# mitake/k8s

Measured on AMD Instinct MI355X. Metric: images/sec ResNet-50 TfJob (train, synthetic ImageNet), higher is better.
Workload: dtype bf16; 1 GPU; model=resnet50-v1.5, global_batch=3072, per_gpu_batch=3072, image_size=224, parallelism=dp1, optimizer=fused SGD momentum 0.9 (HIP)

## Files before the change

k8s_amd/csrc/binding/batchnorm.cpp:

```cpp
#include "binding/common.h"

namespace k8s_amd::binding {
namespace {

int bn_channels(const Tensor& x, const char* name, bool mult8) {
  check_bf16_dense(x, -1, name);
  TORCH_CHECK(x.dim() >= 1 && x.size(-1) > 0, name, ": channels last");
  const int C = (int)x.size(-1);
  TORCH_CHECK(!mult8 || C % 8 == 0, "channels must be a multiple of 8");
  return C;
}
void check_affine(const Tensor& gamma, const Tensor& beta, const Tensor& run_mean, const Tensor& run_var, long C) {
  check_channel_f32(gamma, C, "gamma"); check_channel_f32(beta, C, "beta");
  check_channel_f32(run_mean, C, "run_mean"); check_channel_f32(run_var, C, "run_var");
}
void check_bwd_vectors(const Tensor& mean, const Tensor& invstd, const Tensor& gamma, const Tensor& beta,
                       const Tensor& dgamma, const Tensor& dbeta, long C) {
  check_channel_f32(mean, C, "mean"); check_channel_f32(invstd, C, "invstd");
  check_channel_f32(gamma, C, "gamma"); check_channel_f32(beta, C, "beta");
  check_channel_f32(dgamma, C, "dgamma"); check_channel_f32(dbeta, C, "dbeta");
}
void check_same_shape(const Tensor& t, const Tensor& x, const char* name) {
  check_bf16_dense(t, -1, name);
  TORCH_CHECK(t.sizes() == x.sizes(), name, " must have the shape of x");
}

Tensor relu_mask_for(const Tensor& x, bool want_mask) {
  return want_mask ? torch::empty({x.numel() / 8}, x.options().dtype(at::kByte)) : Tensor();
}

std::vector<Tensor> bn_fwd_impl(const Tensor& x, const OptTensor& res, const Tensor& gamma, const Tensor& beta,
                                const Tensor* sums, const Tensor& run_mean, const Tensor& run_var, bool training,
                                double momentum, double eps, bool relu, bool want_mask, bool want_sub2) {
  const int C = bn_channels(x, "x", true);
  const long M = x.numel() / C;
  check_affine(gamma, beta, run_mean, run_var, C);
  const int nrep = sums ? check_stat_sums(*sums, C, "sums", false) : 0;
  if (res) check_same_shape(*res, x, "res");
  TORCH_CHECK(!want_sub2 || x.dim() == 4, "want_sub2: contiguous NHWC x");
  auto y = torch::empty_like(x);
  auto mean = torch::empty({C}, gamma.options()), invstd = torch::empty({C}, gamma.options());
  auto params = torch::empty({2 * C}, gamma.options());
  Tensor mask = relu_mask_for(x, want_mask);
  uint8_t* mk = want_mask ? mask.data_ptr<uint8_t>() : nullptr;
  std::vector<Tensor> out = {y, mean, invstd};
  if (want_mask) out.push_back(mask);
  if (!sums) {
    Tensor work = training ? torch::empty({k8s_amd::bn_workspace_floats(M, C)}, gamma.options()) : mean;
    launch_bn_fwd(cbf(x), res ? cbf(*res) : nullptr, f32(gamma), f32(beta), bf(y), f32(mean), f32(invstd),
                  f32(run_mean), f32(run_var), f32(work), f32(params), M, C, (float)eps, (float)momentum, training,
                  relu, cur_stream(), mk);
    return out;
  }
  const int H = want_sub2 ? (int)x.size(1) : 1, W = want_sub2 ? (int)x.size(2) : 1;
  Tensor ysub = want_sub2 ? torch::empty({x.size(0), (H + 1) / 2, (W + 1) / 2, C}, x.options()) : Tensor();
  launch_bn_fwd_from_sums(cbf(x), res ? cbf(*res) : nullptr, f32(gamma), f32(beta), bf(y), f32(*sums), nrep, f32(mean),
                          f32(invstd), f32(run_mean), f32(run_var), f32(params), M, C, (float)eps, (float)momentum,
                          relu, cur_stream(), mk, want_sub2 ? bf(ysub) : nullptr, H, W);
  if (want_sub2) out.push_back(ysub);
  return out;
}
std::vector<Tensor> bn_fwd(Tensor x, OptTensor res, Tensor gamma, Tensor beta, Tensor run_mean, Tensor run_var,
                           bool training, double momentum, double eps, bool relu, bool want_mask) {
  return bn_fwd_impl(x, res, gamma, beta, nullptr, run_mean, run_var, training, momentum, eps, relu, want_mask, false);
}
std::vector<Tensor> bn_fwd_from_sums(Tensor x, OptTensor res, Tensor gamma, Tensor beta, Tensor sums, Tensor run_mean,
                                     Tensor run_var, double momentum, double eps, bool relu, bool want_mask,
                                     bool want_sub2) {
  return bn_fwd_impl(x, res, gamma, beta, &sums, run_mean, run_var, true, momentum, eps, relu, want_mask, want_sub2);
}

std::vector<Tensor> bn_fwd_from_sums_dual(Tensor x, Tensor sums, Tensor gamma, Tensor beta, Tensor run_mean,
                                          Tensor run_var, Tensor xr, Tensor sums_r, Tensor gamma_r, Tensor beta_r,
                                          Tensor run_mean_r, Tensor run_var_r, double momentum, double eps) {
  const int C = bn_channels(x, "x", true);
  const long M = x.numel() / C;
  check_same_shape(xr, x, "xr");
  check_affine(gamma, beta, run_mean, run_var, C);
  check_affine(gamma_r, beta_r, run_mean_r, run_var_r, C);
  const int nrep = check_stat_sums(sums, C, "sums", false), nrep_r = check_stat_sums(sums_r, C, "sums_r", false);
  auto y = torch::empty_like(x);
  auto mean = torch::empty({C}, gamma.options()), invstd = torch::empty({C}, gamma.options());
  auto mean_r = torch::empty({C}, gamma.options()), invstd_r = torch::empty({C}, gamma.options());
  auto params = torch::empty({2 * C}, gamma.options()), params_r = torch::empty({2 * C}, gamma.options());
  Tensor mask = relu_mask_for(x, true);
  launch_bn_fwd_from_sums_dual(cbf(x), f32(gamma), f32(beta), f32(sums), nrep, f32(mean), f32(invstd), f32(run_mean),
                               f32(run_var), f32(params), cbf(xr), f32(gamma_r), f32(beta_r), f32(sums_r), nrep_r,
                               f32(mean_r), f32(invstd_r), f32(run_mean_r), f32(run_var_r), f32(params_r), bf(y),
                               mask.data_ptr<uint8_t>(), M, C, (float)eps, (float)momentum, cur_stream());
  return {y, mean, invstd, mask, mean_r, invstd_r};
}

std::vector<Tensor> bn_finalize(Tensor sums, Tensor gamma, Tensor beta, Tensor run_mean, Tensor run_var,
                                int64_t count, double momentum, double eps) {
  const int C = (int)gamma.numel();
  check_affine(gamma, beta, run_mean, run_var, C);
  const int nrep = check_stat_sums(sums, C, "sums", false);
  auto mean = torch::empty({C}, gamma.options()), invstd = torch::empty({C}, gamma.options());
  auto params = torch::empty({2 * C}, gamma.options());
  launch_bn_finalize_sums(f32(gamma), f32(beta), f32(sums), nrep, f32(mean), f32(invstd), f32(run_mean), f32(run_var),
                          f32(params), (long)count, C, (float)eps, (float)momentum, cur_stream());
  return {mean, invstd, params};
}

std::vector<Tensor> bn_relu_maxpool(Tensor x, Tensor sums, Tensor gamma, Tensor beta, Tensor run_mean, Tensor run_var,
                                    double momentum, double eps, bool want_link) {
  check_bf16_dense(x, 4, "x");
  const int N = x.size(0), H = x.size(1), W = x.size(2), C = x.size(3);
  TORCH_CHECK(C > 0 && C % 8 == 0 && 256 % (C / 8) == 0, "C / 8 must divide 256");
  check_affine(gamma, beta, run_mean, run_var, C);
  const int nrep = check_stat_sums(sums, C, "sums", false);
  const int Ho = (H + 1) / 2, Wo = (W + 1) / 2;
  auto y = torch::empty({N, Ho, Wo, C}, x.options());
  auto idx = torch::empty({N, Ho, Wo, C}, x.options().dtype(at::kByte));
  auto mean = torch::empty({C}, gamma.options()), invstd = torch::empty({C}, gamma.options());
  auto params = torch::empty({2 * C}, gamma.options());
  Tensor xarg, ybits;
  if (want_link) {
    xarg = torch::empty({N, Ho, Wo, C}, x.options());
    ybits = torch::empty({(long)N * Ho * Wo * C / 8}, x.options().dtype(at::kByte));
  }
  launch_bn_relu_maxpool_fwd(cbf(x), f32(gamma), f32(beta), f32(sums), nrep, f32(mean), f32(invstd), f32(run_mean),
                             f32(run_var), f32(params), bf(y), idx.data_ptr<uint8_t>(), N, H, W, C, (float)eps,
                             (float)momentum, cur_stream(), want_link ? bf(xarg) : nullptr,
                             want_link ? ybits.data_ptr<uint8_t>() : nullptr);
  if (want_link) return {y, idx, mean, invstd, xarg, ybits};
  return {y, idx, mean, invstd};
}

Tensor pool_bn_bwd_impl(const Tensor& dpool, const Tensor& idx, const Tensor& x, const Tensor& mean,
                        const Tensor& invstd, const Tensor& gamma, const Tensor& beta, const Tensor& dgamma,
                        const Tensor& dbeta, const Tensor* sums) {
  check_bf16_dense(x, 4, "x");
  check_bf16_dense(dpool, 4, "dpool");
  check_cuda(idx, "idx"); check_dtype(idx, at::kByte, "idx");
  const int N = x.size(0), H = x.size(1), W = x.size(2), C = x.size(3);
  TORCH_CHECK(dpool.sizes() == idx.sizes() && dpool.size(0) == N && dpool.size(1) == (H + 1) / 2 &&
                  dpool.size(2) == (W + 1) / 2 && dpool.size(3) == C, "dpool / idx shape mismatch");
  check_bwd_vectors(mean, invstd, gamma, beta, dgamma, dbeta, C);
  const int nrep = sums ? check_stat_sums(*sums, C, "sums", true) : 0;
  auto dx = torch::empty_like(x);
  auto params = torch::empty({4 * C}, gamma.options());
  if (sums) {
    launch_pool_bn_bwd_from_sums(cbf(dpool), idx.data_ptr<uint8_t>(), cbf(x), f32(mean), f32(invstd), f32(gamma),
                                 f32(beta), bf(dx), f32(dgamma), f32(dbeta), f32(*sums), nrep, f32(params), N, H, W, C,
                                 cur_stream());
    return dx;
  }
  auto work = torch::empty({k8s_amd::pool_bn_workspace_floats(C)}, gamma.options());
  launch_pool_bn_bwd(cbf(dpool), idx.data_ptr<uint8_t>(), cbf(x), f32(mean), f32(invstd), f32(gamma), f32(beta), bf(dx),
                     f32(dgamma), f32(dbeta), f32(work), f32(params), N, H, W, C, cur_stream());
  return dx;
}
Tensor pool_bn_bwd_from_sums(Tensor dpool, Tensor idx, Tensor x, Tensor mean, Tensor invstd, Tensor gamma,
                             Tensor beta, Tensor dgamma, Tensor dbeta, Tensor sums) {
  return pool_bn_bwd_impl(dpool, idx, x, mean, invstd, gamma, beta, dgamma, dbeta, &sums);
}
Tensor pool_bn_bwd(Tensor dpool, Tensor idx, Tensor x, Tensor mean, Tensor invstd, Tensor gamma, Tensor beta,
                   Tensor dgamma, Tensor dbeta) {
  return pool_bn_bwd_impl(dpool, idx, x, mean, invstd, gamma, beta, dgamma, dbeta, nullptr);
}

std::vector<Tensor> bn_bwd_impl(const Tensor& dy, const Tensor& x, const OptTensor& y, const Tensor& mean,
                                const Tensor& invstd, const Tensor& gamma, const Tensor& beta, bool relu_x,
                                const Tensor& dgamma, const Tensor& dbeta, bool want_dres, const OptTensor& mask,
                                const Tensor* sums) {
  const int C = bn_channels(x, "x", false);
  const long M = x.numel() / C;
  check_same_shape(dy, x, "dy");
  check_bwd_vectors(mean, invstd, gamma, beta, dgamma, dbeta, C);
  const bool has_mask = mask && mask->defined();
  TORCH_CHECK(!(relu_x && (y || has_mask)) && !(y && has_mask), "relu_x, y and the packed mask are exclusive");
  const uint8_t* mk = has_mask ? check_bit_mask(*mask, x.numel(), "mask") : nullptr;
  const int nrep = sums ? check_stat_sums(*sums, C, "sums", false) : 0;
  Tensor ymask;
  if (y) {
    check_same_shape(*y, x, "y");
    TORCH_CHECK(x.numel() % 8 == 0, "y: a multiple of 8 elements to pack");
    ymask = relu_mask_for(x, true);
    launch_relu_mask(cbf(*y), ymask.data_ptr<uint8_t>(), x.numel() / 8, cur_stream());
    mk = ymask.data_ptr<uint8_t>();
  }
  auto dx = torch::empty_like(x);
  Tensor dres = want_dres ? torch::empty_like(x) : Tensor();
  uint16_t* dr = want_dres ? bf(dres) : nullptr;
  auto params = torch::empty({4 * C}, gamma.options());
  if (sums && mk) {
    launch_bn_bwd_from_sums(cbf(dy), cbf(x), mk, f32(*sums), nrep, f32(mean), f32(invstd), f32(gamma), f32(beta),
                            bf(dx), dr, f32(dgamma), f32(dbeta), f32(params), M, C, cur_stream());
  } else if (sums) {
    launch_bn_bwd_relu_from_sums(cbf(dy), cbf(x), f32(*sums), nrep, f32(mean), f32(invstd), f32(gamma), f32(beta),
                                 bf(dx), f32(dgamma), f32(dbeta), f32(params), M, C, cur_stream());
  } else {
    auto work = torch::empty({k8s_amd::bn_workspace_floats(M, C)}, gamma.options());
    launch_bn_bwd(cbf(dy), cbf(x), f32(mean), f32(invstd), f32(gamma), f32(beta), relu_x, bf(dx), dr, f32(dgamma),
                  f32(dbeta), f32(work), f32(params), M, C, cur_stream(), mk);
  }
  return {dx, dres};
}
std::vector<Tensor> bn_bwd(Tensor dy, Tensor x, OptTensor y, Tensor mean, Tensor invstd, Tensor gamma, Tensor beta,
                           bool relu_x, Tensor dgamma, Tensor dbeta, bool want_dres, OptTensor mask) {
  return bn_bwd_impl(dy, x, y, mean, invstd, gamma, beta, relu_x, dgamma, dbeta, want_dres, mask, nullptr);
}
std::vector<Tensor> bn_bwd_relu_from_sums(Tensor dy, Tensor x, Tensor sums, Tensor mean, Tensor invstd, Tensor gamma,
                                          Tensor beta, Tensor dgamma, Tensor dbeta) {
  return {bn_bwd_impl(dy, x, {}, mean, invstd, gamma, beta, true, dgamma, dbeta, false, {}, &sums)[0]};
}
std::vector<Tensor> bn_bwd_from_sums(Tensor dy, Tensor x, Tensor mask, Tensor sums, Tensor mean, Tensor invstd,
                                     Tensor gamma, Tensor beta, Tensor dgamma, Tensor dbeta, bool want_dres) {
  return bn_bwd_impl(dy, x, {}, mean, invstd, gamma, beta, false, dgamma, dbeta, want_dres, mask, &sums);
}

std::vector<Tensor> bn_bwd_dual_impl(const Tensor& dy, const Tensor& mask, const Tensor& x, const Tensor& mean,
                                     const Tensor& invstd, const Tensor& gamma, const Tensor& beta,
                                     const Tensor& dgamma, const Tensor& dbeta, const Tensor* sums, const Tensor& x2,
                                     const Tensor& mean2, const Tensor& invstd2, const Tensor& gamma2,
                                     const Tensor& beta2, const Tensor& dgamma2, const Tensor& dbeta2,
                                     const Tensor* sums2) {
  const int C = bn_channels(x, "x", !sums);
  const long M = x.numel() / C;
  check_same_shape(dy, x, "dy");
  check_same_shape(x2, x, "x2");
  check_bwd_vectors(mean, invstd, gamma, beta, dgamma, dbeta, C);
  check_bwd_vectors(mean2, invstd2, gamma2, beta2, dgamma2, dbeta2, C);
  const uint8_t* mk = check_bit_mask(mask, x.numel(), "mask");
  const int nrep = sums ? check_stat_sums(*sums, C, "sums", false) : 0;
  TORCH_CHECK(!sums || check_stat_sums(*sums2, C, "sums2", false) == nrep, "sums / sums2: the same replica count");
  auto dx = torch::empty_like(x), dx2 = torch::empty_like(x);
  auto params = torch::empty({4 * C}, gamma.options()), params2 = torch::empty({4 * C}, gamma.options());
  if (sums) {
    launch_bn_bwd_dual_from_sums(cbf(dy), mk, cbf(x), f32(*sums), nrep, f32(mean), f32(invstd), f32(gamma), f32(beta),
                                 bf(dx), f32(dgamma), f32(dbeta), f32(params), cbf(x2), f32(*sums2), f32(mean2),
                                 f32(invstd2), f32(gamma2), f32(beta2), bf(dx2), f32(dgamma2), f32(dbeta2),
                                 f32(params2), M, C, cur_stream());
    return {dx, dx2};
  }
  auto work = torch::empty({k8s_amd::bn_workspace_floats(M, C)}, gamma.options());
  auto work2 = torch::empty({k8s_amd::bn_workspace_floats(M, C)}, gamma.options());
  launch_bn_bwd_dual(cbf(dy), mk, cbf(x), f32(mean), f32(invstd), f32(gamma), f32(beta), bf(dx), f32(dgamma),
                     f32(dbeta), f32(work), f32(params), cbf(x2), f32(mean2), f32(invstd2), f32(gamma2), f32(beta2),
                     bf(dx2), f32(dgamma2), f32(dbeta2), f32(work2), f32(params2), M, C, cur_stream());
  return {dx, dx2};
}
std::vector<Tensor> bn_bwd_dual(Tensor dy, Tensor mask, Tensor x, Tensor mean, Tensor invstd, Tensor gamma,
                                Tensor beta, Tensor dgamma, Tensor dbeta, Tensor x2, Tensor mean2, Tensor invstd2,
                                Tensor gamma2, Tensor beta2, Tensor dgamma2, Tensor dbeta2) {
  return bn_bwd_dual_impl(dy, mask, x, mean, invstd, gamma, beta, dgamma, dbeta, nullptr, x2, mean2, invstd2, gamma2,
                          beta2, dgamma2, dbeta2, nullptr);
}
std::vector<Tensor> bn_bwd_dual_from_sums(Tensor dy, Tensor mask, Tensor x, Tensor mean, Tensor invstd, Tensor gamma,
                                          Tensor beta, Tensor dgamma, Tensor dbeta, Tensor sums, Tensor x2,
                                          Tensor mean2, Tensor invstd2, Tensor gamma2, Tensor beta2, Tensor dgamma2,
                                          Tensor dbeta2, Tensor sums2) {
  return bn_bwd_dual_impl(dy, mask, x, mean, invstd, gamma, beta, dgamma, dbeta, &sums, x2, mean2, invstd2, gamma2,
                          beta2, dgamma2, dbeta2, &sums2);
}

}

void bind_batchnorm(pybind11::module_& m) {
  m.def("bn_fwd", &bn_fwd, "x"_a, "res"_a, "gamma"_a, "beta"_a, "run_mean"_a, "run_var"_a, "training"_a, "momentum"_a,
        "eps"_a, "relu"_a, "want_mask"_a = false);
  m.def("bn_bwd", &bn_bwd, "dy"_a, "x"_a, "y"_a, "mean"_a, "invstd"_a, "gamma"_a, "beta"_a, "relu_x"_a, "dgamma"_a,
        "dbeta"_a, "want_dres"_a, "mask"_a = py::none());
  m.def("bn_fwd_from_sums", &bn_fwd_from_sums, "x"_a, "res"_a, "gamma"_a, "beta"_a, "sums"_a, "run_mean"_a, "run_var"_a,
        "momentum"_a, "eps"_a, "relu"_a, "want_mask"_a = false, "want_sub2"_a = false);
  m.def("bn_bwd_dual", &bn_bwd_dual, "both BatchNorm backwards of bn_fwd_from_sums_dual from one masked dy");
  m.def("bn_fwd_from_sums_dual", &bn_fwd_from_sums_dual, "relu(BN(x) + BN_r(xr)), statistics from conv sums");
  m.def("bn_finalize", &bn_finalize, "sums"_a, "gamma"_a, "beta"_a, "run_mean"_a, "run_var"_a, "count"_a, "momentum"_a,
        "eps"_a);
  m.def("bn_bwd_relu_from_sums", &bn_bwd_relu_from_sums, "relu_x BatchNorm backward from a producer's sums");
  m.def("bn_bwd_from_sums", &bn_bwd_from_sums, "BatchNorm backward from a producer's reduction sums (final + apply)");
  m.def("bn_bwd_dual_from_sums", &bn_bwd_dual_from_sums, "bn_bwd_dual from a producer's reduction sums");
  m.def("bn_relu_maxpool", &bn_relu_maxpool, "x"_a, "sums"_a, "gamma"_a, "beta"_a, "run_mean"_a, "run_var"_a,
        "momentum"_a, "eps"_a, "want_link"_a = false);
  m.def("pool_bn_bwd_from_sums", &pool_bn_bwd_from_sums);
  m.def("pool_bn_bwd", &pool_bn_bwd, "dpool"_a, "idx"_a, "x"_a, "mean"_a, "invstd"_a, "gamma"_a, "beta"_a, "dgamma"_a,
        "dbeta"_a);
}

}
```

k8s_amd/csrc/binding/conv.cpp:

```cpp
#include "binding/common.h"

namespace k8s_amd::binding {
namespace {

int conv_out(int in, int k, int st, int pad, int dil) { return (in + 2 * pad - dil * (k - 1) - 1) / st + 1; }

struct ConvGeom {
  int N, H, W, C, K, R, S;
};
ConvGeom conv_geom(const Tensor& x, const Tensor& w) {
  TORCH_CHECK(x.dim() == 4 && w.dim() == 4, "x [N,H,W,C], w [K,R,S,C]");
  ConvGeom g{(int)x.size(0), (int)x.size(1), (int)x.size(2), (int)x.size(3),
             (int)w.size(0), (int)w.size(1), (int)w.size(2)};
  TORCH_CHECK(w.size(3) == g.C, "channel mismatch");
  TORCH_CHECK(g.C % 8 == 0 && g.K % 8 == 0, "implicit-GEMM conv needs C % 8 == 0 and K % 8 == 0");
  return g;
}
Tensor conv_fwd(Tensor x, Tensor w, int64_t stride, int64_t pad, int64_t dil, bool out_f32, OptTensor bias, int64_t act,
                OptTensor stats, OptTensor xform) {
  check_bf16(x, "x"); check_bf16(w, "w");
  const auto [N, H, W, C, K, R, S] = conv_geom(x, w);
  TORCH_CHECK(stride >= 1 && dil >= 1, "conv_fwd: stride >= 1, dilation >= 1");
  const int Ho = conv_out(H, R, stride, pad, dil), Wo = conv_out(W, S, stride, pad, dil);
  if (bias) check_channel_f32(*bias, K, "bias");
  if (stats) check_stat_sums(*stats, K, "stats", true);
  const float* xf = xform_ptr(xform, C);
  if (xf) TORCH_CHECK(C % 64 == 0 && !out_f32 && !bias && act == 0,
                      "normalize-on-load convolution: C % 64 == 0, bf16 output, no bias / activation");
  auto y = torch::empty({N, Ho, Wo, K}, x.options().dtype(out_f32 ? at::kFloat : at::kBFloat16));
  launch_conv_fwd(cbf(x), cbf(w), y.data_ptr(), out_f32, N, H, W, C, K, R, S, (int)stride, (int)pad, (int)dil, Ho, Wo,
                  optf(bias), (int)act, 0, stats ? f32(*stats) : nullptr, cur_stream(), nullptr, xf);
  return y;
}

Tensor conv_infer(Tensor x, Tensor w, int64_t stride, int64_t pad, Tensor scale, Tensor shift, OptTensor res,
                  bool relu, OptTensor out) {
  check_bf16_dense(x, 4, "x"); check_bf16_dense(w, 4, "w");
  const auto [N, H, W, C, K, R, S] = conv_geom(x, w);
  TORCH_CHECK(stride >= 1 && pad >= 0, "conv_infer: stride >= 1, pad >= 0");
  check_channel_f32(scale, K, "scale"); check_channel_f32(shift, K, "shift");
  TORCH_CHECK(H + 2 * pad >= R && W + 2 * pad >= S, "conv_infer: the filter does not fit the padded image");
  const int Ho = conv_out(H, R, stride, pad, 1), Wo = conv_out(W, S, stride, pad, 1);
  TORCH_CHECK((long)N * Ho * Wo < (1L << 31), "conv_infer: fewer than 2^31 output pixels");
  const std::vector<int64_t> oshape{N, Ho, Wo, K};
  if (out) {
    check_bf16_dense(*out, 4, "out");
    TORCH_CHECK(out->sizes().vec() == oshape, "out must be [N, Ho, Wo, K]");
  }
  if (res) {
    check_bf16_dense(*res, 4, "res");
    TORCH_CHECK(res->sizes().vec() == oshape, "res must have the output's shape [N, Ho, Wo, K]");
  }
  Tensor y = out ? *out : torch::empty(oshape, x.options());
  launch_conv_infer(cbf(x), cbf(w), bf(y), N, H, W, C, K, R, S, (int)stride, (int)pad, Ho, Wo, f32(scale), f32(shift),
                    res ? cbf(*res) : nullptr, relu, cur_stream());
  return y;
}

void conv_fwd_subgrid(Tensor x, Tensor w, int64_t pad, int64_t Hs, int64_t Ws, Tensor out, int64_t stride, int64_t a,
                      int64_t b, bool accumulate, OptTensor bn_x, OptTensor bn_mask, OptTensor bn_mean,
                      OptTensor bn_sums, OptTensor bn_gamma, OptTensor bn_beta, OptTensor bn_invstd) {
  check_bf16(x, "x"); check_bf16(w, "w"); check_bf16(out, "out");
  const auto [N, H, W, C, K, R, S] = conv_geom(x, w);
  TORCH_CHECK(out.dim() == 4 && out.size(0) == N && out.size(3) == K, "out shape");
  const int OH = out.size(1), OW = out.size(2);
  TORCH_CHECK(stride >= 1 && a >= 0 && a < stride && b >= 0 && b < stride, "parity out of range");
  TORCH_CHECK(Hs >= 1 && Ws >= 1 && (Hs - 1) * stride + a < OH && (Ws - 1) * stride + b < OW,
              "sub-grid exceeds the output image");
  k8s_amd::SubGrid sg{OH, OW, (int)stride, (int)a, (int)b};
  k8s_amd::BnBwdSums bb;
  if (bn_sums) {
    TORCH_CHECK(bn_x && bn_mean, "bn sums: bn_x and bn_mean");
    TORCH_CHECK(bn_mask ? accumulate : !accumulate,
                "bn sums: bn_mask + accumulate (a correction) or bn_gamma / bn_beta / bn_invstd + a plain store");
    TORCH_CHECK(bn_x->sizes() == out.sizes(), "bn_x: the shape of out");
    bb = bn_bwd_sums(*bn_x, *bn_mean, *bn_sums, bn_mask, bn_gamma, bn_beta, bn_invstd, {}, {}, {});
  }
  launch_conv_fwd(cbf(x), cbf(w), out.data_ptr(), false, N, H, W, C, K, R, S, 1, (int)pad, 1, (int)Hs, (int)Ws, nullptr,
                  0, accumulate ? 1 : 0, nullptr, cur_stream(), &sg, nullptr, bn_sums ? &bb : nullptr);
}

Tensor conv3x3_dgrad_bnstats(Tensor gy, Tensor wt, Tensor x, Tensor gamma, Tensor beta, Tensor mean, Tensor invstd,
                             Tensor sums) {
  check_bf16_dense(gy, 4, "gy"); check_bf16_dense(wt, 4, "wt"); check_bf16_dense(x, 4, "x");
  const int N = (int)gy.size(0), H = (int)gy.size(1), W = (int)gy.size(2), Kc = (int)gy.size(3);
  const int C = (int)wt.size(0);
  TORCH_CHECK(wt.size(1) == 3 && wt.size(2) == 3 && wt.size(3) == Kc, "wt: [C, 3, 3, K]");
  TORCH_CHECK(x.size(0) == N && x.size(1) == H && x.size(2) == W && x.size(3) == C, "x: the shape of dx");
  TORCH_CHECK(k8s_amd::conv3x3_eligible(H, W, Kc, C, 3, 3, 1, 1, 1), "conv3x3_dgrad_bnstats: outside the kernel");
  const k8s_amd::BnBwdSums bb = bn_bwd_sums(x, mean, sums, {}, gamma, beta, invstd, {}, {}, {});
  Tensor dx = torch::empty({N, H, W, C}, gy.options());
  launch_conv3x3(cbf(gy), cbf(wt), bf(dx), nullptr, nullptr, N, H, W, Kc, C, cur_stream(), &bb);
  return dx;
}

Tensor bwd1x1_fused(Tensor gy, Tensor x, Tensor w, Tensor xform, Tensor gamma, Tensor beta, Tensor mean, Tensor invstd,
                    Tensor dw, Tensor sums, bool accumulate) {
  check_bf16_dense(gy, 2, "gy"); check_bf16_dense(x, 2, "x"); check_bf16_dense(w, 2, "w");
  const long M = gy.size(0), K = gy.size(1), C = x.size(1);
  TORCH_CHECK(x.size(0) == M && w.size(0) == K && w.size(1) == C, "shapes: gy [M, K], x [M, C], w [K, C]");
  TORCH_CHECK(k8s_amd::bwd1x1_fused_ok(M, (int)C, (int)K),
              "bwd1x1_fused: (C, K) = (64, 256) or (128, 512), 1 <= M < 2^31");
  check_cuda(dw, "dw"); check_dtype(dw, at::kFloat, "dw"); check_aligned(dw, "dw");
  TORCH_CHECK(dw.numel() == K * C, "dw must have K * C fp32 elements");
  check_channel_f32(xform, 2 * C, "xform (BatchNorm scale | shift)");
  const k8s_amd::BnBwdSums bb = bn_bwd_sums(x, mean, sums, {}, gamma, beta, invstd, {}, {}, {});
  Tensor dz = torch::empty({M, C}, gy.options());
  launch_bwd1x1_fused(cbf(gy), cbf(x), cbf(w), f32(xform), bb.gamma, bb.beta, bb.mean, bb.invstd, bf(dz), f32(dw),
                      bb.sums, M, (int)C, (int)K, accumulate, cur_stream());
  return dz;
}

void conv_wgrad(Tensor x, Tensor dy, Tensor dw, int64_t stride, int64_t pad, int64_t dil, int64_t splits,
                bool accumulate, OptTensor xform) {
  check_bf16(x, "x"); check_bf16(dy, "dy");
  check_cuda(dw, "dw"); check_dtype(dw, at::kFloat, "dw");
  const auto [N, H, W, C, K, R, S] = conv_geom(x, dw);
  TORCH_CHECK(stride >= 1 && dil >= 1, "conv_wgrad: stride >= 1, dilation >= 1");
  const int Ho = conv_out(H, R, stride, pad, dil), Wo = conv_out(W, S, stride, pad, dil);
  TORCH_CHECK(dy.dim() == 4 && dy.size(0) == N && dy.size(1) == Ho && dy.size(2) == Wo && dy.size(3) == K,
              "dy shape mismatch");
  const float* xf = xform_ptr(xform, C);
  if (dil == 1 && Ho == H && Wo == W && H == W && k8s_amd::wgrad3x3_tiled_ok(C, K, R, S, (int)stride, (int)pad, W)) {
    auto wsp = torch::empty({k8s_amd::wgrad3x3_tiled_workspace(N, H, W, C)}, dw.options());
    launch_wgrad3x3_tiled(cbf(x), cbf(dy), f32(wsp), f32(dw), N, H, W, C, accumulate, cur_stream(), xf);
    return;
  }
  if (!xf && dil == 1 && k8s_amd::wgrad_stream_eligible(N, Ho, Wo, C, K, R, S)) {
    launch_wgrad_stream(cbf(x), cbf(dy), f32(dw), N, H, W, C, K, R, S, (int)stride, (int)pad, Ho, Wo, accumulate,
                        cur_stream());
    return;
  }
  if (xf) TORCH_CHECK(C % 64 == 0, "normalize-on-load weight gradient needs C % 64 == 0");
  int sp = splits <= 0 ? k8s_amd::gemm_choose_splits(K, R * S * C, N * Ho * Wo) : (int)splits;
  Tensor ws;
  if (sp > 1) ws = torch::empty({k8s_amd::gemm_splitk_workspace(K, R * S * C, sp)}, dw.options());
  launch_conv_wgrad(cbf(x), cbf(dy), f32(dw), N, H, W, C, K, R, S, (int)stride, (int)pad, (int)dil, Ho, Wo, sp,
                    accumulate, sp > 1 ? f32(ws) : nullptr, cur_stream(), xf);
}

std::vector<Tensor> conv_dgrad_wsub(Tensor w, std::vector<std::vector<int64_t>> taps) {
  check_bf16(w, "w");
  TORCH_CHECK(w.dim() == 4, "w [K,R,S,C]");
  const int K = w.size(0), R = w.size(1), S = w.size(2), C = w.size(3);
  TORCH_CHECK(!taps.empty() && taps.size() <= 16, "1-16 parities");
  k8s_amd::DgradTaps t{};
  long off = 0;
  std::vector<int64_t> offs;
  for (size_t p = 0; p < taps.size(); ++p) {
    TORCH_CHECK(!taps[p].empty() && taps[p].size() <= 16, "1-16 taps per parity");
    t.n[p] = (int)taps[p].size();
    t.off[p] = off;
    offs.push_back(off);
    for (size_t i = 0; i < taps[p].size(); ++i) {
      TORCH_CHECK(taps[p][i] >= 0 && taps[p][i] < R * S, "tap index out of range");
      t.rs[p][i] = (int)taps[p][i];
    }
    off += (long)C * t.n[p] * K;
    off = (off + 7) / 8 * 8;
  }
  auto out = torch::empty({off}, w.options());
  launch_conv_dgrad_wsub(cbf(w), bf(out), K, R * S, C, t, (int)taps.size(), cur_stream());
  return {out, torch::tensor(offs)};
}
Tensor conv_dgrad_wtrans(Tensor w) {
  check_bf16(w, "w");
  TORCH_CHECK(w.dim() == 4, "w [K,R,S,C]");
  const int K = w.size(0), R = w.size(1), S = w.size(2), C = w.size(3);
  auto w2 = torch::empty({C, R, S, K}, w.options());
  launch_conv_dgrad_wtrans(cbf(w), bf(w2), K, R, S, C, cur_stream());
  return w2;
}

}

void bind_conv(pybind11::module_& m) {
  m.def("conv_fwd", &conv_fwd, "x"_a, "w"_a, "stride"_a, "pad"_a, "dil"_a, "out_f32"_a, "bias"_a, "act"_a, "stats"_a,
        "xform"_a = py::none());
  m.def("conv_infer", &conv_infer, "x"_a, "w"_a, "stride"_a, "pad"_a, "scale"_a, "shift"_a, "res"_a = py::none(),
        "relu"_a = true, "out"_a = py::none());
  m.def("conv3x3_staged_ok", [](int H, int W, int C, int K, int R, int S, int stride, int pad) {
    return k8s_amd::conv3x3_eligible(H, W, C, K, R, S, stride, pad, 1) &&
           k8s_amd::conv3x3_eligible(H, W, K, C, R, S, stride, pad, 1) &&
           k8s_amd::wgrad3x3_tiled_ok(C, K, R, S, stride, pad, W);
  });
  m.def("conv3x3_dgrad_bnstats", &conv3x3_dgrad_bnstats,
        "3x3 stride-1 data gradient with the BatchNorm-backward sums of a relu(BN(x)) input (conv3x3.hip)");
  m.def("conv_fwd_subgrid", &conv_fwd_subgrid, "x"_a, "w"_a, "pad"_a, "Hs"_a, "Ws"_a, "out"_a, "stride"_a, "a"_a, "b"_a,
        "accumulate"_a = false, "bn_x"_a = py::none(), "bn_mask"_a = py::none(), "bn_mean"_a = py::none(),
        "bn_sums"_a = py::none(), "bn_gamma"_a = py::none(), "bn_beta"_a = py::none(), "bn_invstd"_a = py::none());
  m.def("conv_wgrad", &conv_wgrad, "x"_a, "dy"_a, "dw"_a, "stride"_a, "pad"_a, "dil"_a, "splits"_a, "accumulate"_a,
        "xform"_a = py::none());
  m.def("bwd1x1_fused", &bwd1x1_fused, "gy"_a, "x"_a, "w"_a, "xform"_a, "gamma"_a, "beta"_a, "mean"_a, "invstd"_a,
        "dw"_a, "sums"_a, "accumulate"_a,
        "1x1 data gradient, normalize-on-load weight gradient and BatchNorm-backward sums in one pass (bwd1x1_fused.hip)");
  m.def("bwd1x1_fused_ok", [](int64_t M, int64_t C, int64_t K) {
    return C <= 1024 && K <= 4096 && k8s_amd::bwd1x1_fused_ok(M, (int)C, (int)K);
  }, "M"_a, "C"_a, "K"_a, "whether bwd1x1_fused takes this shape");
  m.def("wgrad_stream_eligible",&k8s_amd::wgrad_stream_eligible, "tall-K weight-gradient kernel takes this shape");
  m.def("conv_dgrad_wtrans", &conv_dgrad_wtrans);
  m.def("conv_dgrad_wsub", &conv_dgrad_wsub);
}

}
```

k8s_amd/csrc/kernels/batchnorm.hip:

```cpp
#include <cstdlib>
#include <stdexcept>

#include "common.h"
#include "launchers.h"

namespace k8s_amd {


constexpr int BN_THREADS = 256;

struct BnGeom {
  int cgroups;
  int tpr;
  int rows_per_iter;
  int grid_y;
};

static inline BnGeom bn_geom(int C, long M) {
  BnGeom g;
  g.cgroups = C / 8;
  g.tpr = g.cgroups < BN_THREADS ? g.cgroups : BN_THREADS;
  const long cus = planner_cus();
  long nbx = M / 64;
  nbx = nbx < 1 ? 1 : (nbx > 4 * cus ? 4 * cus : nbx);
// ... 508 lines not shown


__global__ void __launch_bounds__(BN_THREADS) bn_relu_maxpool_fwd_kernel(
    const uint16_t* __restrict__ x, const float* __restrict__ params, uint16_t* __restrict__ y,
    uint8_t* __restrict__ idx, int H, int W, int C, int Ho, int Wo, int total, FastDiv fcv, FastDiv fWo, FastDiv fHo,
    uint16_t* __restrict__ xarg, uint8_t* __restrict__ ybits) {
  const int e = blockIdx.x * BN_THREADS + threadIdx.x;
  if (e >= total) return;
  const int cv = C >> 3;
  const int t = fcv.div(e);
  const int c = (e - t * cv) * 8;
  const int t2 = fWo.div(t);
  const int wo = t - t2 * Wo;
  const int n = fHo.div(t2);
  const int ho = t2 - n * Ho;
  const int h0 = 2 * ho - 1, w0 = 2 * wo - 1;
  float sc[8], sh[8];
  load_f8(params + c, sc);
  load_f8(params + C + c, sh);
  bf16x8_t v[9];
#pragma unroll
  for (int dh = 0; dh < 3; ++dh)
#pragma unroll
    for (int dw = 0; dw < 3; ++dw) {
      const int h = min(max(h0 + dh, 0), H - 1), w = min(max(w0 + dw, 0), W - 1);
      v[dh * 3 + dw] = *reinterpret_cast<const bf16x8_t*>(x + (((long)n * H + h) * W + w) * C + c);
    }
  float best[8];
  uint32_t arg[8];
  bf16x8_t bx = bf16x8_t{0, 0, 0, 0, 0, 0, 0, 0};
#pragma unroll
  for (int j = 0; j < 8; ++j) {
    best[j] = -INFINITY;
    arg[j] = 255;
  }
#pragma unroll
  for (int dh = 0; dh < 3; ++dh)
#pragma unroll
    for (int dw = 0; dw < 3; ++dw) {
      if ((unsigned)(h0 + dh) >= (unsigned)H || (unsigned)(w0 + dw) >= (unsigned)W) continue;
#pragma unroll
      for (int j = 0; j < 8; ++j) {
        const float z = bf2f(f2bf(fmaxf(__builtin_fmaf(bf2f((uint16_t)v[dh * 3 + dw][j]), sc[j], sh[j]), 0.f)));
        if (z > best[j] || (z != z && best[j] == best[j])) {
          best[j] = z;
          arg[j] = (uint32_t)(dh * 3 + dw);
          bx[j] = v[dh * 3 + dw][j];
        }
      }
    }
  store8(y + (long)e * 8, best);
  uint64_t packed = 0;
#pragma unroll
  for (int j = 0; j < 8; ++j) packed |= (uint64_t)arg[j] << (8 * j);
  *reinterpret_cast<uint64_t*>(idx + (long)e * 8) = packed;
  if (xarg) {
    *reinterpret_cast<bf16x8_t*>(xarg + (long)e * 8) = bx;
    uint32_t bits = 0;
#pragma unroll
    for (int j = 0; j < 8; ++j) bits |= (best[j] > 0.f ? 1u : 0u) << j;
    ybits[e] = (uint8_t)bits;
  }
}

struct PoolCell {
  float dz[2][2][8];
};
__device__ __forceinline__ void pool_cell_grad(const uint16_t* __restrict__ dpool, const uint8_t* __restrict__ idx,
                                               int n, int kc, int jc, int c, int C, int Ho, int Wo, PoolCell& pc) {
  uint64_t pk[2][2];
  float g[2][2][8];
#pragma unroll
  for (int a = 0; a < 2; ++a)
#pragma unroll
    for (int b = 0; b < 2; ++b) {
      const bool ok = kc + a < Ho && jc + b < Wo;
      const long o = (((long)n * Ho + (ok ? kc + a : kc)) * Wo + (ok ? jc + b : jc)) * C + c;
      pk[a][b] = ok ? *reinterpret_cast<const uint64_t*>(idx + o) : ~0ull;
      load8(dpool + o, g[a][b]);
    }
#pragma unroll
  for (int dh = 0; dh < 2; ++dh)
#pragma unroll
    for (int dw = 0; dw < 2; ++dw) {
      float acc[8];
#pragma unroll
      for (int r = 0; r < 8; ++r) acc[r] = 0.f;
#pragma unroll
      for (int a = 0; a < 2; ++a)
#pragma unroll
        for (int b = 0; b < 2; ++b) {
          const int oh = dh - 2 * a + 1, ow = dw - 2 * b + 1;
          if (oh < 0 || oh > 2 || ow < 0 || ow > 2) continue;
          const uint32_t pos = (uint32_t)(oh * 3 + ow);
#pragma unroll
          for (int r = 0; r < 8; ++r)
            if (((pk[a][b] >> (8 * r)) & 0xff) == pos) acc[r] += g[a][b][r];
        }
#pragma unroll
      for (int r = 0; r < 8; ++r) pc.dz[dh][dw][r] = bf2f(f2bf(acc[r]));
    }
}

__global__ void __launch_bounds__(BN_THREADS) pool_bn_bwd_reduce_kernel(
    const uint16_t* __restrict__ dpool, const uint8_t* __restrict__ idx, const uint16_t* __restrict__ x,
    const float* __restrict__ mean, const float* __restrict__ invstd, const float* __restrict__ gamma,
    const float* __restrict__ beta, int H, int W, int C, int Ho, int Wo, int Hc, int Wc, int ncells,
    float* __restrict__ part, FastDiv fWc, FastDiv fHc) {
  __shared__ float sh[2][BN_THREADS][9];
  const int t = threadIdx.x, cv = C >> 3;
  const int cg = t % cv, cl = t / cv, cpb = BN_THREADS / cv;
  const int c = cg * 8;
  float sd[8], sx[8], mu[8], is[8], sc[8], bt[8];
#pragma unroll
  for (int j = 0; j < 8; ++j) {
    sd[j] = sx[j] = 0.f;
    mu[j] = mean[c + j];
    is[j] = invstd[c + j];
    bn_affine_regs(gamma[c + j], beta[c + j], mu[j], is[j], sc[j], bt[j]);
  }
  for (int cell = blockIdx.x * cpb + cl; cell < ncells; cell += gridDim.x * cpb) {
    const int r2 = fWc.div(cell), jc = cell - r2 * Wc, n = fHc.div(r2), kc = r2 - n * Hc;
    PoolCell pc;
    pool_cell_grad(dpool, idx, n, kc, jc, c, C, Ho, Wo, pc);
#pragma unroll
    for (int dh = 0; dh < 2; ++dh)
#pragma unroll
      for (int dw = 0; dw < 2; ++dw) {
        const int h = 2 * kc + dh, w = 2 * jc + dw;
        if (h >= H || w >= W) continue;
        const bf16x8_t xv = *reinterpret_cast<const bf16x8_t*>(x + (((long)n * H + h) * W + w) * C + c);
#pragma unroll
        for (int j = 0; j < 8; ++j) {
          const float xf = bf2f((uint16_t)xv[j]);
          const float g = relu_on(xf, sc[j], bt[j]) ? pc.dz[dh][dw][j] : 0.f;
          sd[j] += g;
          sx[j] += g * (xf - mu[j]) * is[j];
        }
      }
  }
#pragma unroll
  for (int j = 0; j < 8; ++j) {
    sh[0][t][j] = sd[j];
    sh[1][t][j] = sx[j];
  }
  __syncthreads();
  if (cl == 0) {
    for (int rr = 1; rr < cpb; ++rr) {
      const int o = rr * cv + cg;
#pragma unroll
      for (int j = 0; j < 8; ++j) {
        sd[j] += sh[0][o][j];
        sx[j] += sh[1][o][j];
      }
    }
#pragma unroll
    for (int j = 0; j < 8; ++j) {
      const long i = ((long)blockIdx.x * C + c + j) * 2;
      part[i] = sd[j];
      part[i + 1] = sx[j];
    }
  }
}

__global__ void __launch_bounds__(BN_THREADS) pool_bn_bwd_apply_kernel(
    const uint16_t* __restrict__ dpool, const uint8_t* __restrict__ idx, const uint16_t* __restrict__ x,
    const float* __restrict__ params, uint16_t* __restrict__ dx, int H, int W, int C, int Ho, int Wo, int total,
    FastDiv fcv, FastDiv fWc, FastDiv fHc) {
  const int e = blockIdx.x * BN_THREADS + threadIdx.x;
  if (e >= total) return;
  const int cv = C >> 3;
  const int t = fcv.div(e);
  const int c = (e - t * cv) * 8;
  const int t2 = fWc.div(t);
  const int jc = t - t2 * (int)fWc.d;
  const int n = fHc.div(t2);
  const int kc = t2 - n * (int)fHc.d;
  PoolCell pc;
  pool_cell_grad(dpool, idx, n, kc, jc, c, C, Ho, Wo, pc);
  float sc[8], B[8], D[8], shf[8];
  load_f8(params + c, sc);
  load_f8(params + C + c, B);
  load_f8(params + 2 * C + c, D);
  load_f8(params + 3 * C + c, shf);
#pragma unroll
  for (int dh = 0; dh < 2; ++dh)
#pragma unroll
    for (int dw = 0; dw < 2; ++dw) {
      const int h = 2 * kc + dh, w = 2 * jc + dw;
      if (h >= H || w >= W) continue;
      const long o = (((long)n * H + h) * W + w) * C + c;
      const bf16x8_t xv = *reinterpret_cast<const bf16x8_t*>(x + o);
      float r[8];
#pragma unroll
      for (int j = 0; j < 8; ++j) {
        const float xf = bf2f((uint16_t)xv[j]);
        const float g = relu_on(xf, sc[j], shf[j]) ? pc.dz[dh][dw][j] : 0.f;
        r[j] = __builtin_fmaf(sc[j], g, __builtin_fmaf(B[j], xf, D[j]));
      }
      store8(dx + o, r);
    }
}

int stream_order_mode() { return 1; }
int stream_dir(int fixed) { return fixed; }

static long bn_rows_per_block(long M, const BnGeom& g) {
  long blocks_x = 4L * planner_cus() / g.grid_y;
  const long cap = M / 64;
  if (blocks_x > cap) blocks_x = cap;
  if (blocks_x < 1) blocks_x = 1;
  long rpb = (M + blocks_x - 1) / blocks_x;
  long minr = (long)g.rows_per_iter * 4;
  if (rpb < minr) rpb = minr;
  rpb = (rpb + g.rows_per_iter - 1) / g.rows_per_iter * g.rows_per_iter;
  return rpb;
}

static int bn_reduce_blocks(long M, const BnGeom& g) {
  long nb = 4L * planner_cus() / g.grid_y;
  const long groups = (M + g.rows_per_iter - 1) / g.rows_per_iter;
  if (nb > groups) nb = groups;
  if (stream_order_mode()) nb = nb < 8 ? 8 : nb & ~7L;
  return (int)(nb < 1 ? 1 : nb);
}

int bn_workspace_floats(long M, int C) {
  BnGeom g = bn_geom(C, M);
  long rpb = bn_rows_per_block(M, g);
  long nb = (M + rpb - 1) / rpb;
  const long nr = bn_reduce_blocks(M, g);
  return (int)((nb > nr ? nb : nr) * C * 2);
}

static void launch_bn_apply(const uint16_t* x, const uint16_t* res, const float* params, uint16_t* y, uint8_t* mask,
                            long M, int C, bool relu, hipStream_t st, const float* rparams = nullptr,
                            uint16_t* ysub = nullptr, int H = 1, int W = 1) {
  const long nvec = M * C / 8;
  if (nvec >= (1L << 31)) throw std::runtime_error("BatchNorm tensor too large (>= 2^31 vectors)");
  if (ysub && (M % ((long)H * W) != 0)) throw std::runtime_error("bn_apply subsample: M must be N * H * W");
  hipLaunchKernelGGL(bn_apply_kernel, dim3(cdiv(nvec, BN_THREADS)), dim3(BN_THREADS), 0, st, x, res, params, rparams,
                     y, mask, (int)nvec, C, make_fastdiv(C / 8), (int)relu,
                     stream_order_mode() ? (stream_dir(1) ? 1 : 2) : 0, ysub, make_fastdiv(W), make_fastdiv(H));
}

void launch_bn_fwd(const uint16_t* x, const uint16_t* res, const float* gamma, const float* beta, uint16_t* y,
                   float* save_mean, float* save_invstd, float* run_mean, float* run_var, float* work, float* params,
                   long M, int C, float eps, float momentum, bool training, bool relu, hipStream_t st,
                   uint8_t* mask) {
  if (training) {
    BnGeom g = bn_geom(C, M);
    long rpb = bn_rows_per_block(M, g);
    int nb = (int)((M + rpb - 1) / rpb);
    hipLaunchKernelGGL(bn_stats_kernel, dim3(nb, g.grid_y), dim3(BN_THREADS), 0, st, x, M, C, g.tpr,
                       g.rows_per_iter, rpb, work);
    hipLaunchKernelGGL(bn_stats_final_kernel, dim3(cdiv(C, FIN_CH)), dim3(256), 0, st, work, nb, M, rpb, C, eps,
                       momentum, save_mean, save_invstd, run_mean, run_var, gamma, beta, params);
  } else {
    hipLaunchKernelGGL(bn_eval_prep_kernel, dim3(cdiv(C, 256)), dim3(256), 0, st, run_mean, run_var, gamma, beta, C,
                       eps, save_mean, save_invstd, params);
  }
  launch_bn_apply(x, res, params, y, mask, M, C, relu, st);
}

void launch_bn_fwd_from_sums(const uint16_t* x, const uint16_t* res, const float* gamma, const float* beta,
                             uint16_t* y, const float* sums, int nrep, float* save_mean, float* save_invstd,
                             float* run_mean, float* run_var, float* params, long M, int C, float eps, float momentum,
                             bool relu, hipStream_t st, uint8_t* mask, uint16_t* ysub, int H, int W) {
  hipLaunchKernelGGL(bn_finalize_sums_kernel, dim3(cdiv(C, 256)), dim3(256), 0, st, sums, nrep, C, (float)M, eps,
                     momentum, save_mean, save_invstd, run_mean, run_var, gamma, beta, params);
  launch_bn_apply(x, res, params, y, mask, M, C, relu, st, nullptr, ysub, H, W);
}

void launch_bn_fwd_from_sums_dual(const uint16_t* x, const float* gamma, const float* beta, const float* sums,
                                  int nrep, float* save_mean, float* save_invstd, float* run_mean, float* run_var,
                                  float* params, const uint16_t* xr, const float* gamma_r, const float* beta_r,
                                  const float* sums_r, int nrep_r, float* save_mean_r, float* save_invstd_r,
                                  float* run_mean_r, float* run_var_r, float* params_r, uint16_t* y, uint8_t* mask,
                                  long M, int C, float eps, float momentum, hipStream_t st) {
  hipLaunchKernelGGL(bn_finalize_sums_kernel, dim3(cdiv(C, 256)), dim3(256), 0, st, sums, nrep, C, (float)M, eps,
                     momentum, save_mean, save_invstd, run_mean, run_var, gamma, beta, params);
  hipLaunchKernelGGL(bn_finalize_sums_kernel, dim3(cdiv(C, 256)), dim3(256), 0, st, sums_r, nrep_r, C, (float)M, eps,
                     momentum, save_mean_r, save_invstd_r, run_mean_r, run_var_r, gamma_r, beta_r, params_r);
  launch_bn_apply(x, xr, params, y, mask, M, C, true, st, params_r);
}

void launch_bn_finalize_sums(const float* gamma, const float* beta, const float* sums, int nrep, float* save_mean,
                             float* save_invstd, float* run_mean, float* run_var, float* params, long M, int C,
                             float eps, float momentum, hipStream_t st) {
  hipLaunchKernelGGL(bn_finalize_sums_kernel, dim3(cdiv(C, 256)), dim3(256), 0, st, sums, nrep, C, (float)M, eps,
                     momentum, save_mean, save_invstd, run_mean, run_var, gamma, beta, params);
}

static void launch_bn_bwd_apply(const uint16_t* dy, const uint16_t* x, const uint8_t* mask, const float* params,
                                bool relu_x, uint16_t* dx, uint16_t* dres, long M, int C, hipStream_t st,
                                int order = -1) {
  const long nvec = M * C / 8;
  if (nvec >= (1L << 31)) throw std::runtime_error("BatchNorm tensor too large (>= 2^31 vectors)");
  if (order < 0) order = stream_order_mode() ? (stream_dir(0) ? 1 : 2) : 0;
  hipLaunchKernelGGL(bn_bwd_apply_kernel, dim3(cdiv(nvec, BN_THREADS)), dim3(BN_THREADS), 0, st, dy, x, mask, params,
                     (int)relu_x, dx, dres, (int)nvec, C, make_fastdiv(C / 8), order);
}

void launch_bn_bwd(const uint16_t* dy, const uint16_t* x, const float* mean, const float* invstd, const float* gamma,
                   const float* beta, bool relu_x, uint16_t* dx, uint16_t* dres, float* dgamma, float* dbeta,
                   float* work, float* params, long M, int C, hipStream_t st, const uint8_t* mask) {
  BnGeom g = bn_geom(C, M);
  const int nb = bn_reduce_blocks(M, g);
  const int rdir = stream_dir(1);
  if (mask)
    hipLaunchKernelGGL(bn_bwd_reduce_kernel<true>, dim3(nb, g.grid_y), dim3(BN_THREADS), 0, st, dy, x, mean, invstd,
                       gamma, beta, (int)relu_x, M, C, g.tpr, g.rows_per_iter, work, mask, rdir);
  else
    hipLaunchKernelGGL(bn_bwd_reduce_kernel<false>, dim3(nb, g.grid_y), dim3(BN_THREADS), 0, st, dy, x, mean, invstd,
                       gamma, beta, (int)relu_x, M, C, g.tpr, g.rows_per_iter, work, mask, rdir);
  hipLaunchKernelGGL(bn_bwd_final_kernel, dim3(cdiv(C, FIN_CH)), dim3(256), 0, st, work, nb, C, dgamma, dbeta,
                     1.f / (float)M, mean, invstd, gamma, beta, params);
  launch_bn_bwd_apply(dy, x, mask, params, relu_x, dx, dres, M, C, st);
}

void launch_bn_bwd_from_sums(const uint16_t* dy, const uint16_t* x, const uint8_t* mask, const float* sums, int nrep,
                             const float* mean, const float* invstd, const float* gamma, const float* beta,
                             uint16_t* dx, uint16_t* dres, float* dgamma, float* dbeta, float* params, long M, int C,
                             hipStream_t st) {
  hipLaunchKernelGGL(bn_bwd_final_sums_kernel, dim3(cdiv(C, 256)), dim3(256), 0, st, sums, sums, nrep, C, dgamma,
                     dbeta, 1.f / (float)M, mean, invstd, gamma, beta, params);
  launch_bn_bwd_apply(dy, x, mask, params, false, dx, dres, M, C, st);
}

void launch_bn_bwd_relu_from_sums(const uint16_t* dy, const uint16_t* x, const float* sums, int nrep,
                                  const float* mean, const float* invstd, const float* gamma, const float* beta,
                                  uint16_t* dx, float* dgamma, float* dbeta, float* params, long M, int C,
                                  hipStream_t st) {
  hipLaunchKernelGGL(bn_bwd_final_sums_kernel, dim3(cdiv(C, 256)), dim3(256), 0, st, sums, sums, nrep, C, dgamma,
                     dbeta, 1.f / (float)M, mean, invstd, gamma, beta, params);
  launch_bn_bwd_apply(dy, x, nullptr, params, true, dx, nullptr, M, C, st);
}

void launch_bn_bwd_dual_from_sums(const uint16_t* dy, const uint8_t* mask, const uint16_t* x, const float* sums,
                                  int nrep, const float* mean, const float* invstd, const float* gamma,
                                  const float* beta, uint16_t* dx, float* dgamma, float* dbeta, float* params,
                                  const uint16_t* x2, const float* sums2, const float* mean2, const float* invstd2,
                                  const float* gamma2, const float* beta2, uint16_t* dx2, float* dgamma2,
                                  float* dbeta2, float* params2, long M, int C, hipStream_t st) {
  hipLaunchKernelGGL(bn_bwd_final_sums_kernel, dim3(cdiv(C, 256)), dim3(256), 0, st, sums, sums, nrep, C, dgamma,
                     dbeta, 1.f / (float)M, mean, invstd, gamma, beta, params);
  hipLaunchKernelGGL(bn_bwd_final_sums_kernel, dim3(cdiv(C, 256)), dim3(256), 0, st, sums, sums2, nrep, C, dgamma2,
                     dbeta2, 1.f / (float)M, mean2, invstd2, gamma2, beta2, params2);
  const long nvec = M * C / 8;
  if (nvec >= (1L << 31)) throw std::runtime_error("BatchNorm tensor too large (>= 2^31 vectors)");
  hipLaunchKernelGGL(bn_bwd_apply_dual_kernel, dim3(cdiv(nvec, BN_THREADS)), dim3(BN_THREADS), 0, st, dy, mask, x,
                     params, dx, x2, params2, dx2, (int)nvec, C, make_fastdiv(C / 8),
                     stream_order_mode() ? (stream_dir(0) ? 1 : 2) : 0);
}

void launch_bn_bwd_dual(const uint16_t* dy, const uint8_t* mask, const uint16_t* x, const float* mean,
                        const float* invstd, const float* gamma, const float* beta, uint16_t* dx, float* dgamma,
                        float* dbeta, float* work, float* params, const uint16_t* x2, const float* mean2,
                        const float* invstd2, const float* gamma2, const float* beta2, uint16_t* dx2, float* dgamma2,
                        float* dbeta2, float* work2, float* params2, long M, int C, hipStream_t st) {
  BnGeom g = bn_geom(C, M);
  const int nb = bn_reduce_blocks(M, g);
  const int rdir = stream_dir(1);
  hipLaunchKernelGGL((bn_bwd_reduce_kernel<true, true>), dim3(nb, g.grid_y), dim3(BN_THREADS), 0, st, dy, x, mean,
                     invstd, gamma, beta, 0, M, C, g.tpr, g.rows_per_iter, work, mask, rdir, x2, mean2, invstd2, work2);
  hipLaunchKernelGGL(bn_bwd_final_kernel, dim3(cdiv(C, FIN_CH)), dim3(256), 0, st, work, nb, C, dgamma, dbeta,
                     1.f / (float)M, mean, invstd, gamma, beta, params);
  hipLaunchKernelGGL(bn_bwd_final_kernel, dim3(cdiv(C, FIN_CH)), dim3(256), 0, st, work2, nb, C, dgamma2, dbeta2,
                     1.f / (float)M, mean2, invstd2, gamma2, beta2, params2);
  const long nvec = M * C / 8;
  if (nvec >= (1L << 31)) throw std::runtime_error("BatchNorm tensor too large (>= 2^31 vectors)");
  hipLaunchKernelGGL(bn_bwd_apply_dual_kernel, dim3(cdiv(nvec, BN_THREADS)), dim3(BN_THREADS), 0, st, dy, mask, x,
                     params, dx, x2, params2, dx2, (int)nvec, C, make_fastdiv(C / 8),
                     stream_order_mode() ? (stream_dir(0) ? 1 : 2) : 0);
}

void launch_bn_relu_maxpool_fwd(const uint16_t* x, const float* gamma, const float* beta, const float* sums, int nrep,
                                float* save_mean, float* save_invstd, float* run_mean, float* run_var, float* params,
                                uint16_t* y, uint8_t* idx, int N, int H, int W, int C, float eps, float momentum,
                                hipStream_t st, uint16_t* xarg, uint8_t* ybits) {
  const int Ho = (H + 1) / 2, Wo = (W + 1) / 2;
  const long total = (long)N * Ho * Wo * (C / 8);
  if ((long)N * H * W * C / 8 >= (1L << 31)) throw std::runtime_error("bn_relu_maxpool: tensor too large");
  hipLaunchKernelGGL(bn_finalize_sums_kernel, dim3(cdiv(C, 256)), dim3(256), 0, st, sums, nrep, C,
                     (float)((long)N * H * W), eps, momentum, save_mean, save_invstd, run_mean, run_var, gamma, beta,
                     params);
  hipLaunchKernelGGL(bn_relu_maxpool_fwd_kernel, dim3(cdiv(total, BN_THREADS)), dim3(BN_THREADS), 0, st, x, params,
                     y, idx, H, W, C, Ho, Wo, (int)total, make_fastdiv(C / 8), make_fastdiv(Wo), make_fastdiv(Ho),
                     xarg, ybits);
}

int pool_bn_workspace_floats(int C) { return 4096 * C * 2; }

void launch_pool_bn_bwd(const uint16_t* dpool, const uint8_t* idx, const uint16_t* x, const float* mean,
                        const float* invstd, const float* gamma, const float* beta, uint16_t* dx, float* dgamma,
                        float* dbeta, float* work, float* params, int N, int H, int W, int C, hipStream_t st) {
  if (C % 8 || BN_THREADS % (C / 8)) throw std::runtime_error("pool_bn_bwd: C / 8 must divide 256");
  const int Ho = (H + 1) / 2, Wo = (W + 1) / 2, Hc = (H + 1) / 2, Wc = (W + 1) / 2;
  const long ncells = (long)N * Hc * Wc;
  if (ncells * (C / 8) >= (1L << 31)) throw std::runtime_error("pool_bn_bwd: tensor too large");
  const int cpb = BN_THREADS / (C / 8);
  long nb = (ncells + cpb - 1) / cpb;
  nb = std::min(nb, 16L * planner_cus());
  hipLaunchKernelGGL(pool_bn_bwd_reduce_kernel, dim3((unsigned)nb), dim3(BN_THREADS), 0, st, dpool, idx, x, mean,
                     invstd, gamma, beta, H, W, C, Ho, Wo, Hc, Wc, (int)ncells, work, make_fastdiv(Wc),
                     make_fastdiv(Hc));
  hipLaunchKernelGGL(bn_bwd_final_kernel, dim3(cdiv(C, FIN_CH)), dim3(256), 0, st, work, (int)nb, C, dgamma, dbeta,
                     1.f / (float)((long)N * H * W), mean, invstd, gamma, beta, params);
  const long total = ncells * (C / 8);
  hipLaunchKernelGGL(pool_bn_bwd_apply_kernel, dim3(cdiv(total, BN_THREADS)), dim3(BN_THREADS), 0, st, dpool, idx, x,
                     params, dx, H, W, C, Ho, Wo, (int)total, make_fastdiv(C / 8), make_fastdiv(Wc),
                     make_fastdiv(Hc));
}

void launch_pool_bn_bwd_from_sums(const uint16_t* dpool, const uint8_t* idx, const uint16_t* x, const float* mean,
                                  const float* invstd, const float* gamma, const float* beta, uint16_t* dx,
                                  float* dgamma, float* dbeta, const float* sums, int nrep, float* params, int N,
                                  int H, int W, int C, hipStream_t st) {
  if (C % 8 || BN_THREADS % (C / 8)) throw std::runtime_error("pool_bn_bwd: C / 8 must divide 256");
  const int Ho = (H + 1) / 2, Wo = (W + 1) / 2, Hc = (H + 1) / 2, Wc = (W + 1) / 2;
  const long ncells = (long)N * Hc * Wc;
  if (ncells * (C / 8) >= (1L << 31)) throw std::runtime_error("pool_bn_bwd: tensor too large");
  hipLaunchKernelGGL(bn_bwd_final_sums_kernel, dim3(cdiv(C, 256)), dim3(256), 0, st, sums, sums, nrep, C, dgamma,
                     dbeta, 1.f / (float)((long)N * H * W), mean, invstd, gamma, beta, params);
  const long total = ncells * (C / 8);
  hipLaunchKernelGGL(pool_bn_bwd_apply_kernel, dim3(cdiv(total, BN_THREADS)), dim3(BN_THREADS), 0, st, dpool, idx, x,
                     params, dx, H, W, C, Ho, Wo, (int)total, make_fastdiv(C / 8), make_fastdiv(Wc),
                     make_fastdiv(Hc));
}

__global__ void __launch_bounds__(BN_THREADS) relu_mask_kernel(const uint16_t* __restrict__ y,
                                                               uint8_t* __restrict__ mask, int nvec) {
  const int e = blockIdx.x * BN_THREADS + threadIdx.x;
  if (e < nvec) mask[e] = relu_bits(*reinterpret_cast<const bf16x8_t*>(y + (long)e * 8));
}

void launch_relu_mask(const uint16_t* y, uint8_t* mask, long nvec, hipStream_t st) {
  if (nvec >= (1L << 31)) throw std::runtime_error("tensor too large (>= 2^31 vectors)");
  hipLaunchKernelGGL(relu_mask_kernel, dim3(cdiv(nvec, BN_THREADS)), dim3(BN_THREADS), 0, st, y, mask, (int)nvec);
}

__global__ void __launch_bounds__(BN_THREADS) mask_apply_kernel(const uint16_t* __restrict__ src,
                                                                const uint8_t* __restrict__ mask,
                                                                uint16_t* __restrict__ out, int nvec) {
  const int e = blockIdx.x * BN_THREADS + threadIdx.x;
  if (e >= nvec) return;
  bf16x8_t v = *reinterpret_cast<const bf16x8_t*>(src + (long)e * 8);
  const uint32_t bits = mask[e];
#pragma unroll
  for (int r = 0; r < 8; ++r) v[r] = ((bits >> r) & 1u) ? v[r] : (short)0;
  *reinterpret_cast<bf16x8_t*>(out + (long)e * 8) = v;
}

void launch_mask_apply(const uint16_t* src, const uint8_t* mask, uint16_t* out, long n, hipStream_t st) {
  if (n % 8) throw std::runtime_error("mask_apply: element count must be a multiple of 8");
  const long nvec = n / 8;
  if (nvec >= (1L << 31)) throw std::runtime_error("tensor too large (>= 2^31 vectors)");
  hipLaunchKernelGGL(mask_apply_kernel, dim3(cdiv(nvec, BN_THREADS)), dim3(BN_THREADS), 0, st, src, mask, out,
                     (int)nvec);
}

}
```

k8s_amd/csrc/kernels/bwd1x1_fused.hip:

```cpp
#include <algorithm>
#include <stdexcept>

#include "common.h"
#include "launchers.h"
#include "mfma.h"

namespace k8s_amd {
namespace b1f {

constexpr int THREADS = 512;
constexpr int CT = 64;

__device__ __attribute__((aligned(64))) uint16_t g_zero16[64];

typedef __attribute__((ext_vector_type(4))) int int4_t;

__device__ __forceinline__ int swz128(int r) { return 2 * (((r >> 1) & 1) | (((r >> 3) & 1) << 1)); }
__device__ __forceinline__ int swz_g(int r) { return (2 * ((r & 3) | (((r >> 3) & 1) << 2))) | ((r >> 2) & 1); }

struct TrRaw {
  short4_t lo, hi;
};
template <int RB, bool G>
__device__ __forceinline__ void tr_load(TrRaw& r, const char* img, int rb, int kk, int lane) {
  const int g = lane >> 4, i = lane & 15, q = i >> 2, p = i & 3;
  const int u = (rb >> 3) + (p >> 1);
  const int r0 = kk * 32 + 8 * g + q, r1 = r0 + 4;
  const int u0 = u ^ (G ? swz_g(r0) : swz128(r0)), u1 = u ^ (G ? swz_g(r1) : swz128(r1));
  tr16_asm(r.lo, img + r0 * RB + (u0 << 4) + (p & 1) * 8);
  tr16_asm(r.hi, img + r1 * RB + (u1 << 4) + (p & 1) * 8);
}
#define K8S_LDS_TIE4(w, a, b, c, d) asm volatile(w : "+v"(a), "+v"(b), "+v"(c), "+v"(d))

struct Args {
  const uint16_t *gy, *x, *w;
  const float *xform, *gamma, *beta, *mean, *invstd;
  uint16_t* dz;
  float* dw;
  float* sums;
  int M, C, ntiles, npairs;
};

__device__ __forceinline__ void lds_barrier() {
  asm volatile("s_waitcnt lgkmcnt(0)" ::: "memory");
  __builtin_amdgcn_s_barrier();
  asm volatile("" ::: "memory");
}

template <int K, int RS, int NSLOT, int HALVES>
__global__ void __launch_bounds__(THREADS, 1) bwd1x1_fused_kernel(Args a) {
  constexpr int RB = K * 2, UG = K / 8;
  constexpr int IMG_G = RS * RB, IMG_X = RS * 128, STAGE = IMG_G + IMG_X, RING = NSLOT * STAGE;
  constexpr int LG = RS * UG / THREADS;
  constexpr int XT = RS * 8;
  constexpr int NKS = K / 32, KW = K / 8, KTW = KW / 16;
  static_assert(LG * THREADS == RS * UG && XT % 64 == 0 && XT <= THREADS && (RS == 32 || RS == 64), "tile");
  static_assert(XT * 64 <= RING, "sums partials reuse the ring");
  constexpr bool PLDS = K > 256;
  __shared__ __attribute__((aligned(1024))) char smem[RING + IMG_X + (PLDS ? 5 * CT * 4 : 0)];
  char* stg = smem + RING;
  float* ptab = reinterpret_cast<float*>(stg + IMG_X);

  const int tid = threadIdx.x, lane = tid & 63;
  const int wid = __builtin_amdgcn_readfirstlane(tid >> 6);
  const int bid = blockIdx.x;
  int pair = bid, chalf = 0;
  if constexpr (HALVES == 2) {
    const int slot = bid >> 3;
    chalf = slot & 1;
    pair = (slot >> 1) * 8 + (bid & 7);
  }
  const int c0 = chalf * CT;
  const int n = pair < a.ntiles ? (a.ntiles - pair + a.npairs - 1) / a.npairs : 0;
  if (n == 0) return;
  const long M = a.M;
  const int C = a.C;

  const int ct = wid & 3, rh = wid >> 2;
  int4_t wf[NKS];
  {
    const uint16_t* wp = a.w + (long)(8 * (lane >> 4)) * C + c0 + ct * 16 + (lane & 15);
#pragma unroll
    for (int ks = 0; ks < NKS; ++ks) {
      bf16x8_t v;
#pragma unroll
      for (int j = 0; j < 8; ++j) v[j] = (short)wp[(long)(ks * 32 + j) * C];
      wf[ks] = __builtin_bit_cast(int4_t, v);
    }
  }
  const int erow = tid >> 3;
  const int eu = (tid & 7) ^ swz128(erow);
  const int ecol = c0 + eu * 8;
  float xsc[8], xsh[8], gsc[8], gsh[8], mu[8], ps[8], pq[8];
#pragma unroll
  for (int j = 0; j < 8; ++j) {
    xsc[j] = a.xform[ecol + j];
    xsh[j] = a.xform[C + ecol + j];
    mu[j] = a.mean[ecol + j];
    bn_affine_regs(a.gamma[ecol + j], a.beta[ecol + j], mu[j], a.invstd[ecol + j], gsc[j], gsh[j]);
    ps[j] = pq[j] = 0.f;
  }
  if constexpr (PLDS) {
    if (tid < 8) {
#pragma unroll
      for (int j = 0; j < 8; ++j) {
        ptab[0 * CT + tid * 8 + j] = xsc[j];
        ptab[1 * CT + tid * 8 + j] = xsh[j];
        ptab[2 * CT + tid * 8 + j] = gsc[j];
        ptab[3 * CT + tid * 8 + j] = gsh[j];
        ptab[4 * CT + tid * 8 + j] = mu[j];
      }
    }
  }
#pragma unroll
  for (int ks = 0; ks < NKS; ++ks) asm volatile("" : "+v"(wf[ks]));
  if constexpr (!PLDS) {
#pragma unroll
    for (int j = 0; j < 8; ++j) asm volatile("" : "+v"(xsc[j]), "+v"(xsh[j]), "+v"(gsc[j]), "+v"(gsh[j]), "+v"(mu[j]));
  } else {
    __syncthreads();
  }

  auto issue = [&](int slot, int i) {
    char* st = smem + slot * STAGE;
    const long m0 = (long)(pair + i * a.npairs) * RS;
#pragma unroll
    for (int j = 0; j < LG; ++j) {
      const int sl = j * THREADS + tid, row = sl / UG, up = sl % UG;
      const int u = up ^ swz_g(row);
      const long m = m0 + row;
      const void* src = m < M ? (const void*)(a.gy + m * K + u * 8) : (const void*)g_zero16;
      glds16(src, st + j * (THREADS * 16) + wid * 1024);
    }
    if (wid < XT / 64) {
      const long m = m0 + erow;
      const void* src = m < M ? (const void*)(a.x + m * C + ecol) : (const void*)g_zero16;
      glds16(src, st + IMG_G + wid * 1024);
    }
  };

  f32x4_t dwa[KTW][4];
#pragma unroll
  for (int i = 0; i < KTW; ++i)
#pragma unroll
    for (int j = 0; j < 4; ++j) dwa[i][j] = f32x4_t{0.f, 0.f, 0.f, 0.f};

  const int pre = min(n, NSLOT - 1);
  for (int s = 0; s < pre; ++s) issue(s, s);
  int slot = 0;
  for (int s = 0; s < n; ++s) {
    const int younger = min(n - 1, s + NSLOT - 2) - s;
    if (younger >= 2) asm volatile("s_waitcnt vmcnt(%0)" ::"n"(2 * LG) : "memory");
    else if (younger == 1) asm volatile("s_waitcnt vmcnt(%0)" ::"n"(LG) : "memory");
    else asm volatile("s_waitcnt vmcnt(0)" ::: "memory");
    lds_barrier();
    if (s + NSLOT - 1 < n) issue(slot == 0 ? NSLOT - 1 : slot - 1, s + NSLOT - 1);
    char* G = smem + slot * STAGE;
    char* X = G + IMG_G;

    {
      f32x4_t d0 = {0.f, 0.f, 0.f, 0.f}, d1 = {0.f, 0.f, 0.f, 0.f};
      const int row0 = rh * (RS / 2) + (lane & 15);
      const int kq = lane >> 4;
      if constexpr (RS == 64) {
        const int row1 = row0 + 16;
        const char* p0 = G + row0 * RB;
        const char* p1 = G + row1 * RB;
        const int s0 = swz_g(row0), s1 = swz_g(row1);
#pragma unroll
        for (int ks = 0; ks < NKS; ++ks) {
          const bf16x8_t b0 = *reinterpret_cast<const bf16x8_t*>(p0 + (((ks * 4 + kq) ^ s0) << 4));
          const bf16x8_t b1 = *reinterpret_cast<const bf16x8_t*>(p1 + (((ks * 4 + kq) ^ s1) << 4));
          const mfma_bf16x8 wa = __builtin_bit_cast(mfma_bf16x8, wf[ks]);
          d0 = mfma16(wa, __builtin_bit_cast(mfma_bf16x8, b0), d0);
          d1 = mfma16(wa, __builtin_bit_cast(mfma_bf16x8, b1), d1);
        }
      } else {
        const char* p0 = G + row0 * RB;
        const int s0 = swz_g(row0);
#pragma unroll
        for (int ks = 0; ks < NKS; ks += 2) {
          const bf16x8_t b0 = *reinterpret_cast<const bf16x8_t*>(p0 + (((ks * 4 + kq) ^ s0) << 4));
          const bf16x8_t b1 = *reinterpret_cast<const bf16x8_t*>(p0 + (((ks * 4 + 4 + kq) ^ s0) << 4));
          d0 = mfma16(__builtin_bit_cast(mfma_bf16x8, wf[ks]), __builtin_bit_cast(mfma_bf16x8, b0), d0);
          d1 = mfma16(__builtin_bit_cast(mfma_bf16x8, wf[ks + 1]), __builtin_bit_cast(mfma_bf16x8, b1), d1);
        }
        d0 += d1;
      }
      const int unit = ct * 2 + (lane >> 5), half = (lane >> 4) & 1;
      auto put = [&](int row, const f32x4_t& d) {
        bf16x4_t o;
#pragma unroll
        for (int r = 0; r < 4; ++r) o[r] = (short)f2bf(d[r]);
        *reinterpret_cast<bf16x4_t*>(stg + row * 128 + ((unit ^ swz128(row)) << 4) + half * 8) = o;
      };
      put(row0, d0);
      if constexpr (RS == 64) put(row0 + 16, d1);
    }
    lds_barrier();

    if (wid < XT / 64) {
      const bf16x8_t dzv = *reinterpret_cast<const bf16x8_t*>(stg + tid * 16);
      const bf16x8_t xv = *reinterpret_cast<const bf16x8_t*>(X + tid * 16);
      if constexpr (PLDS) {
        const float* t = ptab + (ecol - c0);
#pragma unroll
        for (int j = 0; j < 8; ++j) {
          xsc[j] = t[j];
          xsh[j] = t[CT + j];
          gsc[j] = t[2 * CT + j];
          gsh[j] = t[3 * CT + j];
          mu[j] = t[4 * CT + j];
        }
      }
      float o[8];
#pragma unroll
      for (int j = 0; j < 8; ++j) {
        const float xf = bf2f((uint16_t)xv[j]);
        o[j] = fmaxf(__builtin_fmaf(xf, xsc[j], xsh[j]), 0.f);
        const float g = relu_on(xf, gsc[j], gsh[j]) ? bf2f((uint16_t)dzv[j]) : 0.f;
        ps[j] += g;
        pq[j] = __builtin_fmaf(g, xf - mu[j], pq[j]);
      }
      *reinterpret_cast<bf16x8_t*>(X + tid * 16) = pack_bf16x8(o);
      const long m = (long)(pair + s * a.npairs) * RS + erow;
      if (m < M) *reinterpret_cast<bf16x8_t*>(a.dz + m * C + ecol) = dzv;
    }
    lds_barrier();

#pragma unroll
    for (int kk = 0; kk < RS / 32; ++kk) {
      TrRaw ar[KTW], br[4];
#pragma unroll
      for (int j = 0; j < 4; ++j) tr_load<128, false>(br[j], X, j * 16, kk, lane);
#pragma unroll
      for (int i = 0; i < KTW; ++i) tr_load<RB, true>(ar[i], G, wid * KW + i * 16, kk, lane);
      K8S_LDS_TIE8("s_waitcnt lgkmcnt(0)", br[0].lo, br[0].hi, br[1].lo, br[1].hi, br[2].lo, br[2].hi, br[3].lo,
                   br[3].hi);
#pragma unroll
      for (int i = 0; i < KTW; i += 2)
        K8S_LDS_TIE4("s_waitcnt lgkmcnt(0)", ar[i].lo, ar[i].hi, ar[i + 1].lo, ar[i + 1].hi);
#pragma unroll
      for (int i = 0; i < KTW; ++i)
#pragma unroll
        for (int j = 0; j < 4; ++j)
          dwa[i][j] = __builtin_amdgcn_mfma_f32_16x16x32_bf16(join8(br[j].lo, br[j].hi), join8(ar[i].lo, ar[i].hi),
                                                              dwa[i][j], 0, 0, 0);
    }
    slot = slot + 1 == NSLOT ? 0 : slot + 1;
  }

#pragma unroll
  for (int i = 0; i < KTW; ++i) {
    const int k = wid * KW + i * 16 + (lane & 15);
#pragma unroll
    for (int j = 0; j < 4; ++j) {
      float* d = a.dw + (long)k * C + c0 + j * 16 + 4 * (lane >> 4);
#pragma unroll
      for (int r = 0; r < 4; ++r) atomicAdd(d + r, dwa[i][j][r]);
    }
  }
  __syncthreads();
  float* part = reinterpret_cast<float*>(smem);
  if (tid < XT) {
#pragma unroll
    for (int j = 0; j < 8; ++j) {
      part[tid * 16 + j] = ps[j];
      part[tid * 16 + 8 + j] = pq[j];
    }
  }
  __syncthreads();
  if (tid < 2 * CT) {
    const int col = tid & (CT - 1), which = tid / CT;
    const int u = col >> 3, r = col & 7;
    float v = 0.f;
#pragma unroll 4
    for (int row = 0; row < RS; ++row) v += part[(row * 8 + (u ^ swz128(row))) * 16 + which * 8 + r];
    atomicAdd(a.sums + (long)(bid % kConvStatReplicas) * 2 * C + (long)which * C + c0 + col, v);
  }
}

}

bool bwd1x1_fused_ok(long M, int C, int K) {
  return M >= 1 && M < (1L << 31) && ((C == 64 && K == 256) || (C == 128 && K == 512));
}

void launch_bwd1x1_fused(const uint16_t* gy, const uint16_t* x, const uint16_t* w, const float* xform,
                         const float* gamma, const float* beta, const float* mean, const float* invstd, uint16_t* dz,
                         float* dw, float* sums, long M, int C, int K, bool accumulate, hipStream_t st) {
  using namespace b1f;
  if (!bwd1x1_fused_ok(M, C, K)) throw std::runtime_error("bwd1x1_fused: (C, K) = (64, 256) or (128, 512), M < 2^31");
  if (!accumulate) (void)hipMemsetAsync(dw, 0, (size_t)K * C * sizeof(float), st);
  Args a{gy, x, w, xform, gamma, beta, mean, invstd, dz, dw, sums, (int)M, C, 0, 0};
  const int cus = std::max(1, planner_cus());
  if (C == 64) {
    a.ntiles = (int)((M + 63) / 64);
    a.npairs = cus;
    hipLaunchKernelGGL((bwd1x1_fused_kernel<256, 64, 3, 1>), dim3(cus), dim3(THREADS), 0, st, a);
  } else {
    const int grid = std::max(16, cus / 16 * 16);
    a.ntiles = (int)((M + 31) / 32);
    a.npairs = grid / 2;
    hipLaunchKernelGGL((bwd1x1_fused_kernel<512, 32, 4, 2>), dim3(grid), dim3(THREADS), 0, st, a);
  }
}

}
```

k8s_amd/csrc/kernels/launchers.h:

```cpp
#pragma once
#include <hip/hip_runtime.h>
#include <stdint.h>

#include "rng.h"

namespace k8s_amd {

int planner_cus();
void set_planner_cus(int n);

void launch_sgd(float* p, float* mom, const void* g, bool g_bf16, uint16_t* pbf, long n, const uint8_t* decay_mask, float lr,
                float mu, float wd, float scale, const float* scale_ptr, const float* hyper, bool nesterov,
                bool first_step, hipStream_t st);
void launch_adam(float* p, float* m1, float* m2, const void* g, bool g_bf16, uint16_t* pbf, long n, const uint8_t* decay_mask,
                 float lr, float b1, float b2, float eps, float wd, float scale, const float* scale_ptr,
                 const float* hyper, float bc1, float bc2, bool decoupled, hipStream_t st);
void launch_sumsq(const void* g, bool g_bf16, long n, float* out, hipStream_t st);
void launch_clip_factor(const float* stats, float max_norm, float* factor, hipStream_t st);
void launch_slice_sum(const uint16_t* in, long n, int world, float* out, uint16_t* out_bf, hipStream_t st);
void launch_cast_bf16(const float* in, uint16_t* out, long n, hipStream_t st);

void launch_grad_accumulate(float* acc, const float* g, long n, bool first, hipStream_t st);
void launch_grad_fold(float* g, const float* acc, uint16_t* out_bf, long n, hipStream_t st);

constexpr int kLayerItemMax = 16384;
void launch_layer_sums(const long* items, int n_items, const float* p, float* m1, float* m2, const void* g,
                       bool g_bf16, const uint8_t* flags, float* partial, bool lamb, float b1, float b2, float eps,
                       float wd, float scale, const float* scale_ptr, const float* hyper, float bc1, float bc2,
                       hipStream_t st);
void launch_layer_fold(const float* partial, const int* seg_start, int n_seg, float* sums, const float* scale_ptr,
                       hipStream_t st);
void launch_layer_ratio(const float* sums, const uint8_t* flags, int n_seg, float* ratio, bool lamb, float eta,
                        float wd, const float* scale_ptr, hipStream_t st);
void launch_layer_update(const long* items, int n_items, float* p, float* m1, const float* m2, const void* g,
                         bool g_bf16, uint16_t* pbf, const uint8_t* flags, const float* ratio, bool lamb, float lr,
                         float mu, float b1, float b2, float eps, float wd, float scale, const float* scale_ptr,
                         const float* hyper, float bc1, float bc2, bool first_step, hipStream_t st);

int bn_workspace_floats(long M, int C);
void launch_bn_fwd(const uint16_t* x, const uint16_t* res, const float* gamma, const float* beta, uint16_t* y,
                   float* save_mean, float* save_invstd, float* run_mean, float* run_var, float* work, float* params,
                   long M, int C, float eps, float momentum, bool training, bool relu, hipStream_t st,
                   uint8_t* mask = nullptr);
void launch_bn_fwd_from_sums(const uint16_t* x, const uint16_t* res, const float* gamma, const float* beta,
                             uint16_t* y, const float* sums, int nrep, float* save_mean, float* save_invstd,
                             float* run_mean, float* run_var, float* params, long M, int C, float eps, float momentum,
                             bool relu, hipStream_t st, uint8_t* mask = nullptr, uint16_t* ysub = nullptr,
                             int H = 1, int W = 1);
void launch_bn_fwd_from_sums_dual(const uint16_t* x, const float* gamma, const float* beta, const float* sums,
                                  int nrep, float* save_mean, float* save_invstd, float* run_mean, float* run_var,
                                  float* params, const uint16_t* xr, const float* gamma_r, const float* beta_r,
                                  const float* sums_r, int nrep_r, float* save_mean_r, float* save_invstd_r,
                                  float* run_mean_r, float* run_var_r, float* params_r, uint16_t* y, uint8_t* mask,
                                  long M, int C, float eps, float momentum, hipStream_t st);
void launch_bn_bwd_from_sums(const uint16_t* dy, const uint16_t* x, const uint8_t* mask, const float* sums, int nrep,
                             const float* mean, const float* invstd, const float* gamma, const float* beta,
                             uint16_t* dx, uint16_t* dres, float* dgamma, float* dbeta, float* params, long M, int C,
                             hipStream_t st);
void launch_bn_bwd_relu_from_sums(const uint16_t* dy, const uint16_t* x, const float* sums, int nrep,
                                  const float* mean, const float* invstd, const float* gamma, const float* beta,
                                  uint16_t* dx, float* dgamma, float* dbeta, float* params, long M, int C,
                                  hipStream_t st);
void launch_bn_bwd_dual_from_sums(const uint16_t* dy, const uint8_t* mask, const uint16_t* x, const float* sums,
                                  int nrep, const float* mean, const float* invstd, const float* gamma,
                                  const float* beta, uint16_t* dx, float* dgamma, float* dbeta, float* params,
                                  const uint16_t* x2, const float* sums2, const float* mean2, const float* invstd2,
                                  const float* gamma2, const float* beta2, uint16_t* dx2, float* dgamma2,
                                  float* dbeta2, float* params2, long M, int C, hipStream_t st);
void launch_bn_bwd_dual(const uint16_t* dy, const uint8_t* mask, const uint16_t* x, const float* mean,
                        const float* invstd, const float* gamma, const float* beta, uint16_t* dx, float* dgamma,
                        float* dbeta, float* work, float* params, const uint16_t* x2, const float* mean2,
                        const float* invstd2, const float* gamma2, const float* beta2, uint16_t* dx2, float* dgamma2,
                        float* dbeta2, float* work2, float* params2, long M, int C, hipStream_t st);
void launch_bn_finalize_sums(const float* gamma, const float* beta, const float* sums, int nrep, float* save_mean,
                             float* save_invstd, float* run_mean, float* run_var, float* params, long M, int C,
                             float eps, float momentum, hipStream_t st);
constexpr int kConvStatReplicas = 32;
void launch_bn_bwd(const uint16_t* dy, const uint16_t* x, const float* mean, const float* invstd, const float* gamma,
                   const float* beta, bool relu_x, uint16_t* dx, uint16_t* dres, float* dgamma, float* dbeta,
                   float* work, float* params, long M, int C, hipStream_t st, const uint8_t* mask = nullptr);
void launch_relu_mask(const uint16_t* y, uint8_t* mask, long nvec, hipStream_t st);

void launch_norm_fwd(bool rms, const uint16_t* x, const uint16_t* res, uint16_t* xsum, const float* gamma,
                     const float* beta, uint16_t* y, float* mean, float* rstd, long R, int D, float eps,
                     hipStream_t st, const DropArgs* drop = nullptr);
int norm_workspace_floats(long R, int D);
void launch_norm_bwd(bool rms, const uint16_t* dy, const uint16_t* x, const float* gamma, const float* mean,
                     const float* rstd, const uint16_t* dres, uint16_t* dx, float* dgamma, float* dbeta, float* work,
                     long R, int D, hipStream_t st, float* dsum = nullptr, const DropArgs* drop = nullptr,
                     uint16_t* da = nullptr);

void launch_dropout(const uint16_t* x, uint16_t* y, long R, int D, const DropArgs& dr, hipStream_t st);
void launch_dropout_mask(uint8_t* out, long row0, long R, int C, const DropArgs& dr, hipStream_t st);

void launch_xent_fwd(const void* logits, bool bf16, const int64_t* labels, long R, long V, long ld, float* loss,
                     float* lse, long ignore_index, float smoothing, hipStream_t st);
void launch_xent_bwd(const void* logits, bool bf16, const int64_t* labels, const float* lse, const float* dscale,
                     bool per_row, long R, long V, long ld, void* dlogits, long ignore_index, float smoothing,
                     hipStream_t st);
void launch_xent_eval(const void* logits, bool bf16, const int64_t* labels, long R, long V, long ld, float* loss,
                      int* rank, long ignore_index, hipStream_t st);

int gemm_choose_splits(int M, int N, int K);
struct AddEpi {
  const uint16_t* src;
  const uint8_t* mask;
};
bool gemm_short_ok(int M, int N, int K, long lda, long ldc);
bool gemm_short_bnstats_ok(int M, int N, int K, bool dual);
struct BnBwdSums {
  const uint16_t* x = nullptr;
  const float* gamma = nullptr;
  const float* beta = nullptr;
  const float* mean = nullptr;
  const float* invstd = nullptr;
  float* sums = nullptr;
  const uint8_t* mask = nullptr;
  const uint16_t* x2 = nullptr;
  const float* mean2 = nullptr;
  float* sums2 = nullptr;
};
struct GemmShortBnStats {
  const uint16_t* x = nullptr;
  const uint8_t* mask = nullptr;
  const float* mean = nullptr;
  float* sums = nullptr;
  const uint16_t* x2 = nullptr;
  const float* mean2 = nullptr;
  float* sums2 = nullptr;
};
void launch_gemm_short(const uint16_t* A, const uint16_t* B, long ldb, bool b_mn, uint16_t* C, const uint16_t* add,
                       const uint8_t* mask, const float* xf, float* stats, int M, int N, int K, int epi,
                       hipStream_t st, const GemmShortBnStats* bst = nullptr);
void launch_gemm_dgrad_bnstats(const uint16_t* A, const uint16_t* B, uint16_t* C, int M, int N, int K,
                               const BnBwdSums& bb, hipStream_t st, bool accumulate = false,
                               const uint16_t* add_src = nullptr, const uint8_t* add_mask = nullptr);
void launch_gemm(const uint16_t* A, long lda, bool a_kmajor, const uint16_t* B, long ldb, bool b_kmajor, void* C,
                 long ldc, bool c_f32, int M, int N, int K, const float* bias, int act, uint16_t* pre, int mode,
                 float alpha, int splits, float* ws, hipStream_t st, const AddEpi* add = nullptr,
                 const float* xform_b = nullptr, int xform_c = 0);
void launch_mask_apply(const uint16_t* src, const uint8_t* mask, uint16_t* out, long n, hipStream_t st);
long gemm_splitk_workspace(int M, int N, int splits);
bool conv3x3_eligible(int H, int W, int C, int K, int R, int S, int stride, int pad, int dil);
void launch_conv3x3(const uint16_t* x, const uint16_t* w, uint16_t* y, float* stats, const float* xform, int N,
                    int H, int W, int C, int K, hipStream_t st,
                    const BnBwdSums* bsums = nullptr);
bool gemm256_eligible(int M, int N, int K, bool a_kmajor, bool b_kmajor);
int gemm256_choose_splits(int M, int N, int K);
bool gemm_w4_dact_ok(int M, int N, int K, long lda, long ldb, long ldc);
long gemm_w4_dact_part_floats(int M, int N);
void launch_gemm_w4_dact(const uint16_t* A, long lda, const uint16_t* B, long ldb, uint16_t* C, long ldc, int M, int N,
                         int K, const uint16_t* pre, int act, float* part, float* db, bool db_accumulate,
                         float* sk_slabs, int* sk_sync, hipStream_t st);
bool gemm_w4_swiglu_ok(int M, int F, int K, long lda, long ldb);
void launch_gemm_w4_swiglu_bwd(const uint16_t* A, long lda, const uint16_t* B, long ldb, uint16_t* dgu,
                               const uint16_t* gu, int M, int F, int K, int blk, float* sk_slabs, int* sk_sync,
                               hipStream_t st);
bool gemm_w4_stats_ok(int M, int N, int K);
bool gemm_w4_dgrad_bnstats_ok(int M, int N, int K);
void launch_gemm_w4_dgrad_bnstats(const uint16_t* A, const uint16_t* B, uint16_t* y, int M, int N, int K,
                                  const uint16_t* x, const float* tab, float* sums, float* sk_slabs, int* sk_sync,
                                  hipStream_t st);
void launch_gemm_w4_stats(const uint16_t* A, long lda, const uint16_t* B, long ldb, uint16_t* y, int M, int N, int K,
                          float* stats, float* sk_slabs, int* sk_sync, hipStream_t st);
bool gemm_w4_rope_ok(int M, int N, int K, long lda, long ldb, int rot_cols);
void launch_gemm_w4_rope(const uint16_t* A, long lda, const uint16_t* B, long ldb, uint16_t* y, int M, int N, int K,
                         const int* pos, const float* table, int rot_cols, float* sk_slabs, int* sk_sync,
                         hipStream_t st);
bool gemm_w4_swiglu_fwd_ok(int M, int F, int K, long lda, long ldb);
void launch_gemm_w4_swiglu_fwd(const uint16_t* A, long lda, const uint16_t* B, long ldb, uint16_t* gu, uint16_t* h,
                               int M, int F, int K, float* sk_slabs, int* sk_sync, hipStream_t st);
struct Gemm256Plan {
  int tiles, full, sk, kps;
};
Gemm256Plan gemm256_plan(int M, int N, int K);
long gemm256_sk_slab_floats(const Gemm256Plan& p);
long gemm256_sk_sync_ints(const Gemm256Plan& p);
void launch_gemm256(const uint16_t* A, long lda, bool a_kmajor, const uint16_t* B, long ldb, bool b_kmajor, void* C,
                    long ldc, bool c_f32, int M, int N, int K, const float* bias, int act, uint16_t* pre,
                    bool accumulate, float alpha, hipStream_t st, int splits = 1, float* ws = nullptr,
                    float* sk_slabs = nullptr, int* sk_sync = nullptr);
struct SubGrid {
  int H, W, stride, a, b;
};
void launch_conv_fwd(const uint16_t* x, const uint16_t* w, void* y, bool y_f32, int N, int H, int W, int C, int K,
                     int R, int S, int stride, int pad, int dil, int Ho, int Wo, const float* bias, int act,
                     int mode, float* stats, hipStream_t st, const SubGrid* sg = nullptr, const float* xform = nullptr,
                     const BnBwdSums* bb = nullptr);
void launch_conv_infer(const uint16_t* x, const uint16_t* w, uint16_t* y, int N, int H, int W, int C, int K, int R,
                       int S, int stride, int pad, int Ho, int Wo, const float* scale, const float* shift,
                       const uint16_t* res, bool relu, hipStream_t st);
void launch_conv_wgrad(const uint16_t* x, const uint16_t* dy, float* dw, int N, int H, int W, int C, int K, int R,
                       int S, int stride, int pad, int dil, int Ho, int Wo, int splits, bool accumulate, float* ws,
                       hipStream_t st, const float* xform = nullptr);
bool wgrad_stream_eligible(int N, int Ho, int Wo, int C, int K, int R, int S);
void launch_wgrad_stream(const uint16_t* x, const uint16_t* dy, float* dw, int N, int H, int W, int C, int K, int R,
                         int S, int stride, int pad, int Ho, int Wo, bool accumulate, hipStream_t st);
bool bwd1x1_fused_ok(long M, int C, int K);
void launch_bwd1x1_fused(const uint16_t* gy, const uint16_t* x, const uint16_t* w, const float* xform,
                         const float* gamma, const float* beta, const float* mean, const float* invstd, uint16_t* dz,
                         float* dw, float* sums, long M, int C, int K, bool accumulate, hipStream_t st);
void launch_conv_dgrad_wtrans(const uint16_t* w, uint16_t* w2, int K, int R, int S, int C, hipStream_t st);
struct DgradTaps {
  int n[16];
  long off[16];
  int rs[16][16];
};
void launch_conv_dgrad_wsub(const uint16_t* w, uint16_t* out, int K, int RS, int C, const DgradTaps& taps, int np,
                            hipStream_t st);

void launch_swiglu_fwd(const uint16_t* gu, uint16_t* y, long T, int F, int blk, hipStream_t st);
void launch_swiglu_bwd(const uint16_t* gu, const uint16_t* dy, uint16_t* dgu, long T, int F, int blk, hipStream_t st);
void launch_rope(uint16_t* x, long ld, const int* pos, const float* table, long T, int H, int D, bool inverse,
                 hipStream_t st);
void launch_gelu_bwd(const uint16_t* dy, const uint16_t* pre, uint16_t* dx, long n, hipStream_t st);
void launch_relu_bwd(const uint16_t* dy, const uint16_t* y, uint16_t* dx, long n, hipStream_t st);
int colsum_workspace_floats(long R, int C);
void launch_colsum(const uint16_t* x, long R, int C, float* work, float* out, bool accumulate, hipStream_t st);
void launch_colsum_fold(float* part, int P, int C, float* out, bool accumulate, hipStream_t st);
void launch_colsum_group(float* part, int P, int C, int gs, hipStream_t st);
void launch_act_bwd_colsum(int act, const uint16_t* dy, const uint16_t* pre, uint16_t* g, long R, int C, float* work,
                           float* out, bool accumulate, hipStream_t st);

struct AttnFwdArgs {
  const uint16_t *q, *k, *v;
  uint16_t* o;
  float* lse;
  const int* kv_lens;
  long sqb, sqs, sqh, skb, sks, skh, svb, svs, svh, sob, sos, soh;
  long lse_ld;
  int B, Sq, Sk, Hq, Hkv, causal;
  float scale_log2;
  DropArgs drop;
};
struct AttnBwdArgs {
  const uint16_t *q, *k, *v, *dO;
  const float* lse;
  float* delta;
  uint16_t* dq;
  uint16_t *dk, *dv;
  const int* kv_lens;
  long sqb, sqs, sqh, skb, sks, skh, svb, svs, svh, sdb, sds, sdh;
  long sgqb, sgqs, sgqh, sgkb, sgks, sgkh, sgvb, sgvs, sgvh;
  long lse_ld;
  int B, Sq, Sk, Hq, Hkv, causal;
  float scale_log2, scale;
  int dkv_split = 1;
  float* dkv_ws = nullptr;
  float* cpart = nullptr;
  int cpart_ld = 0;
  DropArgs drop;
};
int flash_dkv_splits(int B, int Sq, int Sk, int Hkv, int causal);
bool flash_bwd_one_block(int D, int Sq, int Sk, int Hq, int Hkv, int dkv_split);
void launch_bn_relu_maxpool_fwd(const uint16_t* x, const float* gamma, const float* beta, const float* sums, int nrep,
                                float* save_mean, float* save_invstd, float* run_mean, float* run_var, float* params,
                                uint16_t* y, uint8_t* idx, int N, int H, int W, int C, float eps, float momentum,
                                hipStream_t st, uint16_t* xarg = nullptr, uint8_t* ybits = nullptr);
void launch_pool_bn_bwd_from_sums(const uint16_t* dpool, const uint8_t* idx, const uint16_t* x, const float* mean,
                                  const float* invstd, const float* gamma, const float* beta, uint16_t* dx,
                                  float* dgamma, float* dbeta, const float* sums, int nrep, float* params, int N,
                                  int H, int W, int C, hipStream_t st);
int pool_bn_workspace_floats(int C);
void launch_pool_bn_bwd(const uint16_t* dpool, const uint8_t* idx, const uint16_t* x, const float* mean,
                        const float* invstd, const float* gamma, const float* beta, uint16_t* dx, float* dgamma,
                        float* dbeta, float* work, float* params, int N, int H, int W, int C, hipStream_t st);

int stream_order_mode();
int stream_dir(int fixed);

void launch_flash_fwd(const AttnFwdArgs& a, int D, hipStream_t st);
void launch_flash_bwd(const AttnBwdArgs& a, int D, const uint16_t* o, long sob, long sos, long soh, hipStream_t st);

struct EmbTable {
  const uint16_t* w;
  float* g;
  const int64_t* ids;
  int V;
};
void launch_embed_fwd(const EmbTable* tabs, int ntab, int T, int D, int S, uint16_t* out, hipStream_t st);
void launch_embed_bwd(const EmbTable* tabs, int ntab, int T, int D, int S, const uint16_t* g, hipStream_t st);

void launch_avgpool_fwd(const uint16_t* x, uint16_t* y, int N, int HW, int C, hipStream_t st);
void launch_avgpool_bwd(const uint16_t* dy, uint16_t* dx, int N, int HW, int C, hipStream_t st);

void launch_stem_s2d_input(const uint16_t* x, int N, int H, int W, int Cin, int pad, uint16_t* out, hipStream_t st);
void launch_stem_w_s2d(const uint16_t* w7, int K, int R, int Cw, uint16_t* w4, hipStream_t st);
bool stem_conv_fwd_ok(int K, int R, int C, int Wo);
void launch_stem_conv_fwd(const uint16_t* xs, const uint16_t* w4, uint16_t* y, float* stats, int N, int Hs, int Ws,
                          hipStream_t st);
void splitk_reduce(const float* ws, int splits, long mn, float* out, bool accumulate, hipStream_t st);
bool wgrad3x3_tiled_ok(int C, int K, int R, int S, int stride, int pad, int W);
int wgrad3x3_tiled_blocks(int N, int H, int W, int C);
long wgrad3x3_tiled_workspace(int N, int H, int W, int C);
void launch_wgrad3x3_tiled(const uint16_t* x, const uint16_t* dy, float* ws, float* dw, int N, int H, int W, int C,
                           bool accumulate, hipStream_t st, const float* xform = nullptr);
int stem_wgrad_blocks(int N, int Hs);
void launch_stem_wgrad(const uint16_t* xs, const uint16_t* dy, float* ws, float* dw4, int N, int Hs, int Ws,
                       hipStream_t st);
void launch_stem_dw_s2d(const float* dw4, int K, int R, int Cw, float* dw7, hipStream_t st);

void launch_subsample_nhwc(const uint16_t* x, uint16_t* y, int N, int H, int W, int C, int s, hipStream_t st);
void launch_maxpool_fwd(const uint16_t* x, uint16_t* y, uint8_t* idx, int N, int H, int W, int C, int Ho, int Wo,
                        int k, int s, int p, hipStream_t st);
void launch_maxpool_bwd(const uint16_t* dy, const uint8_t* idx, uint16_t* dx, int N, int H, int W, int C, int Ho,
                        int Wo, int k, int s, int p, hipStream_t st);

}
```

k8s_amd/models/resnet.py:

```python
from __future__ import annotations

import math
from typing import List

import torch
import torch.nn as nn

from k8s_amd.ops import nn as K
from k8s_amd.parallel.flat import ParamStore, init_const, init_kaiming_normal, init_uniform


class BN(nn.Module):
    def __init__(self, store: ParamStore, name: str, c: int, zero_init: bool = False):
        super().__init__()
        self.gamma = store.new(name + ".weight", (c,), init_const(0.0 if zero_init else 1.0), decay=False, lowp=False)
        self.beta = store.new(name + ".bias", (c,), init_const(0.0), decay=False, lowp=False)
        self.register_buffer("running_mean", torch.zeros(c))
        self.register_buffer("running_var", torch.ones(c))
        self.momentum, self.eps = 0.1, 1e-5

    def forward(self, x, residual=None, relu=True, res_link=None, dy_link=None, sub2=False):
        sums = None
        if isinstance(x, tuple):
            x, sums = x
        return K.batch_norm_act(x, self.gamma, self.beta, self.running_mean, self.running_var, residual, relu,
                                self.training, self.momentum, self.eps, sums=sums, res_link=res_link,
                                dy_link=dy_link, sub2=sub2)


class Conv(nn.Module):
    def __init__(self, store: ParamStore, name: str, cin: int, cout: int, k: int, stride: int = 1):
        super().__init__()
        self.w = store.new(name + ".weight", (cout, k, k, cin), init_kaiming_normal(cin * k * k))
        self.stride, self.pad = stride, k // 2

    def forward(self, x, grad_link=None):
        return K.conv2d_nhwc(x, self.w, self.stride, self.pad, with_stats=True, grad_link=grad_link)


class Bottleneck(nn.Module):
    expansion = 4

    def __init__(self, store, name, cin, width, stride, downsample):
        super().__init__()
        cout = width * 4
        self.conv1 = Conv(store, name + ".conv1", cin, width, 1)
        self.bn1 = BN(store, name + ".bn1", width)
        self.conv2 = Conv(store, name + ".conv2", width, width, 3, stride)
        self.bn2 = BN(store, name + ".bn2", width)
        self.conv3 = Conv(store, name + ".conv3", width, cout, 1)
        self.bn3 = BN(store, name + ".bn3", cout, zero_init=True)
        self.down = None
        if downsample:
            self.down = Conv(store, name + ".downsample.0", cin, cout, 1, stride)
            self.down_bn = BN(store, name + ".downsample.1", cout)

    def forward(self, x, sub2=False):
        idn = x
        identity = self.down is None and x.requires_grad
        link = K.GradLink() if identity else None
        dlink = K.GradLink(shared=True) if (self.down is not None and x.requires_grad) else None
        mlink = dn = None
        if self.down is not None:
            mlink = K.MaskLink()
            dn = self.down(x, grad_link=dlink)
            fuse = K.BN_DUAL and isinstance(dn, tuple) and dn[1] is not None and self.training and dn[0].is_cuda
            if not fuse:
                idn = self.down_bn(dn, relu=False, dy_link=mlink)
        t = self.conv1(x, grad_link=link or dlink)
        t = K.bn_relu_conv(t, self.bn1, self.conv2)
        t = K.bn_relu_conv(t, self.bn2, self.conv3)
        if dn is not None and fuse:
            y = K.bn_act_dual(t, self.bn3, dn, self.down_bn)
            if y is not None:
                return y
            idn = self.down_bn(dn, relu=False, dy_link=mlink)
        return self.bn3(t, residual=idn, relu=True, res_link=link or mlink, sub2=sub2)


class ResNet(nn.Module):
    def __init__(self, store: ParamStore, layers: List[int] = (3, 4, 6, 3), num_classes: int = 1000,
                 in_ch: int = 3, width: int = 64, stem_s2d: bool = True):
        super().__init__()
        self.store = store
        self.stem_s2d = stem_s2d
        self.in_ch = in_ch
        self.stem_ch = (in_ch + 7) // 8 * 8
        self.conv1 = Conv(store, "conv1", self.stem_ch, width, 7, 2)
        self.bn1 = BN(store, "bn1", width)
        blocks = []
        cin = width
        for i, n in enumerate(layers):
            w = width * (2 ** i)
            for j in range(n):
                stride = 2 if (j == 0 and i > 0) else 1
                blocks.append(Bottleneck(store, "layer%d.%d" % (i + 1, j), cin, w, stride, j == 0))
                cin = w * 4
        self.blocks = nn.ModuleList(blocks)
        self.fc_w = store.new("fc.weight", (num_classes, cin), init_uniform(1.0 / math.sqrt(cin)))
        self.fc_b = store.new("fc.bias", (num_classes,), init_uniform(1.0 / math.sqrt(cin)), decay=False,
                              lowp=False)
        self.num_classes = num_classes

    def finalize(self, device, **kw):
        self.store.finalize(device, **kw)
        if self.stem_ch != self.in_ch:
            with torch.no_grad():
                self.conv1.w.master[..., self.in_ch:].zero_()
            self.store.refresh_lowp()
        return self.to(device)

    def prepare_input(self, images_nhwc: torch.Tensor, s2d: bool = None) -> torch.Tensor:
        use = self.stem_s2d if s2d is None else s2d
        if use and images_nhwc.is_cuda and images_nhwc.dtype == torch.bfloat16 and self.conv1.w.shape[1] == 7:
            return K.stem_s2d_input(images_nhwc, pad=3)
        if images_nhwc.shape[-1] == self.stem_ch:
            return images_nhwc
        pad = self.stem_ch - images_nhwc.shape[-1]
        return torch.nn.functional.pad(images_nhwc, (0, pad))

    def forward(self, x):
        if x.shape[-1] == 16 and self.stem_s2d and x.is_cuda:
            t = K.stem_conv_s2d(x, self.conv1.w)
        else:
            t = self.conv1(x)
        y = K.bn_relu_maxpool(t, self.bn1)
        for i, b in enumerate(self.blocks):
            nxt = self.blocks[i + 1] if i + 1 < len(self.blocks) else None
            y = b(y, sub2=nxt is not None and nxt.down is not None and nxt.down.stride == 2)
        y = K.global_avg_pool_nhwc(y)
        return K.linear(y, self.fc_w, self.fc_b)

    def batch_norms(self):
        out = [self.bn1]
        for b in self.blocks:
            out += [b.bn1, b.bn2, b.bn3] + ([b.down_bn] if b.down is not None else [])
        return out

    def folded_views(self, flat: torch.Tensor):
        views, off = [], 0
        for bn in self.batch_norms():
            c = bn.running_mean.numel()
            views.append((flat[off:off + c], flat[off + c:off + 2 * c]))
            off += 2 * c
        assert off == flat.numel(), "folded BatchNorm tensor of another model"
        return views

    @torch.no_grad()
    def fold_bn(self):
        bns = self.batch_norms()
        dev = self.bn1.running_mean.device
        flat = torch.empty(2 * sum(bn.running_mean.numel() for bn in bns), device=dev, dtype=torch.float32)
        views = self.folded_views(flat)
        for bn, (scale, shift) in zip(bns, views):
            torch.mul(bn.gamma.master.float(), torch.rsqrt(bn.running_var.float() + bn.eps), out=scale)
            torch.sub(bn.beta.master.float(), bn.running_mean.float() * scale, out=shift)
        return flat, views

    @torch.no_grad()
    def forward_infer(self, x, folded=None):
        if folded is None:
            folded = self.fold_bn()
        views = self.folded_views(folded) if torch.is_tensor(folded) else folded[1]
        it = iter(views)
        sc, sh = next(it)
        if x.shape[-1] == 16 and self.stem_s2d and x.is_cuda:
            t = K.stem_conv_s2d(x, self.conv1.w)[0]
            bn = self.bn1
            t = K.batch_norm_act(t, bn.gamma, bn.beta, bn.running_mean, bn.running_var, None, True, False,
                                 bn.momentum, bn.eps)
        else:
            t = K.conv_bn_act_infer(x, self.conv1.w, sc, sh, self.conv1.stride, self.conv1.pad)
        y = K.max_pool_nhwc(t, 3, 2, 1)
        for b in self.blocks:
            (s1, h1), (s2, h2), (s3, h3) = next(it), next(it), next(it)
            idn = y
            if b.down is not None:
                sd, hd = next(it)
                idn = K.conv_bn_act_infer(y, b.down.w, sd, hd, b.down.stride, b.down.pad, relu=False)
            t = K.conv_bn_act_infer(y, b.conv1.w, s1, h1, b.conv1.stride, b.conv1.pad)
            t = K.conv_bn_act_infer(t, b.conv2.w, s2, h2, b.conv2.stride, b.conv2.pad)
            y = K.conv_bn_act_infer(t, b.conv3.w, s3, h3, b.conv3.stride, b.conv3.pad, residual=idn)
        y = K.global_avg_pool_nhwc(y)
        return K.linear(y, self.fc_w, self.fc_b)


def resnet50(store: ParamStore, num_classes: int = 1000) -> ResNet:
    return ResNet(store, (3, 4, 6, 3), num_classes)


def resnet_tiny(store: ParamStore, num_classes: int = 10) -> ResNet:
    return ResNet(store, (1, 1, 1, 1), num_classes, width=8)
```

k8s_amd/ops/conv.py:

```python
from __future__ import annotations

import collections
import os
import warnings

import torch
import torch.nn.functional as F

from k8s_amd.ops._ext import load as _load



STATS = {"hip_fwd": 0, "aten_fwd": 0, "hip_wgrad": 0, "aten_wgrad": 0, "hip_dgrad": 0, "aten_dgrad": 0,
         "bn_bstats": 0, "hip_infer": 0, "aten_infer": 0}
ROUTES = collections.Counter()



def _nchw(x):
    return x.permute(0, 3, 1, 2)


def _nhwc(y):
    return y.permute(0, 2, 3, 1).contiguous()


def _hip(*ts):
    return all(t.is_cuda and t.dtype == torch.bfloat16 for t in ts)


def fwd_ok(x, w):
    return _hip(x, w) and x.shape[-1] % 8 == 0 and w.shape[0] % 8 == 0


def _key(op, x, w, stride, padding):
    return "%s|%s|%s|%d|%d" % (op, "x".join(map(str, x.shape)), "x".join(map(str, w.shape)), stride, padding)


def fwd_uses_hip(x, w, stride, padding) -> bool:
    return fwd_ok(x, w)


_WARNED = set()


def _vendor(op, x, w, stride, padding):
    if x.is_cuda:
        STATS["aten_" + op] += 1
        key = _key("conv_" + op, x, w, stride, padding)
        if key not in _WARNED:
            _WARNED.add(key)
            warnings.warn("k8s_amd conv: %s is outside the MFMA kernels' shape contract; using ATen" % key)


def conv_fwd(x, w, stride, padding, stats=None):
    if fwd_uses_hip(x, w, stride, padding):
        STATS["hip_fwd"] += 1
        return _load().conv_fwd(x, w, stride, padding, 1, False, None, 0, stats)
    _vendor("fwd", x, w, stride, padding)
    return _nhwc(F.conv2d(_nchw(x), _nchw(w), None, stride, padding))


def infer_ok(x, w, scale, shift, residual=None) -> bool:
    ts = [x, w] + ([residual] if residual is not None else [])
    return (_hip(*ts) and x.shape[-1] % 8 == 0 and w.shape[0] % 8 == 0
            and all(t.is_contiguous() and t.data_ptr() % 16 == 0 for t in ts)
            and scale.is_cuda and shift.is_cuda and scale.dtype == torch.float32 and shift.dtype == torch.float32
            and scale.is_contiguous() and shift.is_contiguous())


def conv_infer(x, w, stride, padding, scale, shift, residual=None, relu=True):
    if infer_ok(x, w, scale, shift, residual):
        STATS["hip_infer"] += 1
        return _load().conv_infer(x, w, stride, padding, scale, shift, residual, relu)
    _vendor("infer", x, w, stride, padding)
    y = F.conv2d(_nchw(x), _nchw(w), None, stride, padding).permute(0, 2, 3, 1)
    y = (y.float() * scale.float() + shift.float()).to(x.dtype)
    if residual is not None:
        y = y.float() + residual.float()
    if relu:
        y = torch.relu(y)
    return y.to(x.dtype).contiguous()


def _aten_bwd(gy, x, w, stride, padding, need_dx, need_dw):
    dx, dw, _ = torch.ops.aten.convolution_backward(
        _nchw(gy), _nchw(x), _nchw(w), None, [stride, stride], [padding, padding], [1, 1], False, [0, 0], 1,
        [bool(need_dx), bool(need_dw), False])
    return (_nhwc(dx) if dx is not None else None), (dw.permute(0, 2, 3, 1) if dw is not None else None)


def _wgrad_hip(C_, gy, x, out, stride, padding, acc, xform=None):
    K, R, S, C = out.shape
    N, Ho, Wo = gy.shape[0], gy.shape[1], gy.shape[2]
    if (R == 1 and S == 1 and stride == 1 and padding == 0
            and (xform is not None or not C_.wgrad_stream_eligible(N, Ho, Wo, C, K, R, S))):
        C_.gemm(gy.reshape(-1, K), False, x.reshape(-1, C), False, out.view(K, C), True, None, 0, None, acc, 1.0, 0,
                xform_b=xform, xform_c=C if xform is not None else 0)
    else:
        C_.conv_wgrad(x, gy, out, stride, padding, 1, 0, acc, xform=xform)


BSTATS_3X3 = os.environ.get("K8S_AMD_BN_BSTATS_3X3", "1") != "0"
BSTATS_GEMM = os.environ.get("K8S_AMD_BN_BSTATS_GEMM", "1") != "0"
BSTATS_ENTRY = os.environ.get("K8S_AMD_BN_BSTATS_ENTRY", "1") != "0"
BSTATS_TILE_MASK = os.environ.get("K8S_AMD_BN_BSTATS_TILE_MASK", "1") != "0"
BSTATS_STRIDED = os.environ.get("K8S_AMD_BN_BSTATS_STRIDED", "0") != "0"
BSTATS_TILE_SHORT = os.environ.get("K8S_AMD_BN_BSTATS_TILE_SHORT", "0") != "0"


def _bn_sums(C_, bn_link, C, device):
    R = C_.conv_stat_replicas
    if bn_link.store is not None:
        from k8s_amd.ops.nn import _zero_scratch
        return _zero_scratch(bn_link.store, device, R * 2 * C).view(R, 2, C)
    return torch.zeros(R, 2, C, device=device, dtype=torch.float32)


def _link_kind(bn_link, shape):
    filled = bn_link is not None and bn_link.kind is not None and bn_link.x.shape == shape
    return bn_link.kind if filled else None


def _plan_dgrad(C_, gy, w, padding, addend, bn_link):
    K, R, S, C = w.shape
    N, Ho, Wo = gy.shape[:3]
    masked = addend is not None and not torch.is_tensor(addend)
    kind = _link_kind(bn_link, (N, Ho + R - 1 - 2 * padding, Wo + S - 1 - 2 * padding, C))
    if (BSTATS_3X3 and kind == "relu" and addend is None and R == 3 and S == 3 and padding == 1 and Ho == Wo
            and C_.conv3x3_staged_ok(Ho, Wo, C, K, 3, 3, 1, 1)):
        return "conv3x3_relu_sums"
    if not (R == 1 and S == 1 and padding == 0):
        return "implicit_flipped"
    M = N * Ho * Wo
    if masked:
        residual = kind in ("mask", "dual", "pool")
        if residual and C_.gemm_short_bnstats_ok(M, C, K, kind == "dual"):
            return "short_mask_sums"
        if (residual and BSTATS_TILE_MASK and M < 2 ** 31
                and (BSTATS_TILE_SHORT or kind != "dual" or not C_.gemm_short_bnstats_ok(M, C, K, False))):
            return "tile_mask_sums"
        return "gemm_masked_add"
    if addend is None:
        if BSTATS_GEMM and kind == "relu" and C_.gemm_dgrad_bnstats_ok(M, C, K):
            return "tile_relu_sums"
        if BSTATS_ENTRY and kind == "mask" and C_.gemm_short_bnstats_ok(M, C, K, False):
            return "short_entry_pending"
        return "gemm_plain"
    if kind == "pool" and addend.is_contiguous() and C % 8 == 0 and M < 2 ** 31:
        return "tile_final_sums"
    return "gemm_add"


def _dgrad_hip(C_, gy, w, padding, addend=None, bn_link=None):
    route = _plan_dgrad(C_, gy, w, padding, addend, bn_link)
    ROUTES[route] += 1
    K, R, S, C = w.shape
    ln = bn_link
    if route == "implicit_flipped":
        if addend is not None and not torch.is_tensor(addend):
            addend = addend.materialize()
        dx = C_.conv_fwd(gy, C_.conv_dgrad_wtrans(w), 1, R - 1 - padding, 1, False, None, 0, None)
        return dx if addend is None else dx.add_(addend)
    if route == "conv3x3_relu_sums":
        sums = _bn_sums(C_, ln, C, gy.device)
        dx = C_.conv3x3_dgrad_bnstats(gy, C_.conv_dgrad_wtrans(w), ln.x, ln.gamma, ln.beta, ln.mean, ln.invstd, sums)
        ln.deposit(sums, None, dx)
        return dx
    shape = gy.shape[:3] + (C,)
    gy, w = gy.reshape(-1, K), w.reshape(K, C)
    if route == "gemm_plain":
        return C_.gemm(gy, True, w, False, None, False, None, 0, None, False, 1.0, 1).reshape(shape)
    if route == "gemm_add":
        C_.gemm(gy, True, w, False, addend.view(-1, C), False, None, 0, None, True, 1.0, 1)
        return addend
    if route == "gemm_masked_add":
        out = torch.empty(shape, device=gy.device, dtype=gy.dtype)
        C_.gemm(gy, True, w, False, out.view(-1, C), False, None, 0, None, True, 1.0, 1,
                add_src=addend.dy.view(-1, C), add_mask=addend.mask)
        return out
    sums, sums2, x = _bn_sums(C_, ln, C, gy.device), None, ln.x.view(-1, C)
    if route == "tile_relu_sums":
        out = C_.gemm_dgrad_bnstats(gy, w, x, ln.gamma, ln.beta, ln.mean, ln.invstd, sums).view(shape)
    elif route == "short_entry_pending":
        out = C_.dgrad_short_bnstats(gy, w, None, None, x, ln.mask, ln.mean, sums).view(shape)
        ln.deposit_pending(sums)
        return out
    elif route == "tile_final_sums":
        out = addend
        C_.gemm_dgrad_bnstats_mask(gy, w, out.view(-1, C), x, ln.mask, ln.mean, sums)
    else:
        x2 = None
        if ln.kind == "dual":
            sums2, x2 = _bn_sums(C_, ln, C, gy.device), ln.x2.view(-1, C)
        add = addend.dy.view(-1, C)
        if route == "short_mask_sums":
            out = C_.dgrad_short_bnstats(gy, w, add, addend.mask, x, ln.mask, ln.mean, sums, x2, ln.mean2,
                                         sums2).view(shape)
        else:
            out = torch.empty(shape, device=gy.device, dtype=gy.dtype)
            C_.gemm_dgrad_bnstats_mask(gy, w, out.view(-1, C), x, ln.mask, ln.mean, sums, add, addend.mask, x2,
                                       ln.mean2, sums2)
    ln.deposit(sums, sums2, out)
    return out


def _parity_taps(R, a, pad, stride):
    taps = sorted(((a + pad - r) // stride, r) for r in range(R) if (a + pad - r) % stride == 0)
    if taps and [d for d, _ in taps] != list(range(taps[0][0], taps[0][0] + len(taps))):
        return None
    return taps


def strided_dgrad_ok(gy, w, stride, padding):
    K, R, S, C = w.shape
    if stride < 2 or K % 8 or C % 8:
        return False
    for a in range(stride):
        for b in range(stride):
            tr, ts = _parity_taps(R, a, padding, stride), _parity_taps(S, b, padding, stride)
            if tr is None or ts is None:
                return False
            if tr and ts and tr[0][0] != ts[0][0]:
                return False
    return True


def _plan_dgrad_strided(gy, w, stride, padding, H, W, addend, bn_link):
    K, R, S, C = w.shape
    kind = _link_kind(bn_link, (gy.shape[0], H, W, C))
    if bn_link is not None and bn_link.pending:
        if (kind is not None and R == 1 and S == 1 and padding == 0 and torch.is_tensor(addend)
                and addend.is_contiguous() and addend.shape == bn_link.x.shape):
            return "parity_complete_sums"
        bn_link.drop_pending()
    if BSTATS_STRIDED and kind == "relu" and addend is None and C > 64 and K % 64 == 0:
        return "parity_relu_sums"
    return "parity"


def _dgrad_strided_hip(C_, gy, w, stride, padding, H, W, addend=None, bn_link=None):
    route = _plan_dgrad_strided(gy, w, stride, padding, H, W, addend, bn_link)
    ROUTES[route] += 1
    K, R, S, C = w.shape
    ln = bn_link
    tail = (addend is not None,)
    if route == "parity_complete_sums":
        tail = (True, ln.x, ln.mask, ln.mean, ln.sums)
    elif route == "parity_relu_sums":
        rsums = _bn_sums(C_, ln, C, gy.device)
        tail = (False, ln.x, None, ln.mean, rsums, ln.gamma, ln.beta, ln.invstd)
    live = [(a, b, _parity_taps(R, a, padding, stride), _parity_taps(S, b, padding, stride))
            for a in range(stride) for b in range(stride)]
    live = [(a, b, tr, ts) for a, b, tr, ts in live if tr and ts]
    if addend is not None:
        dx = addend
    else:
        alloc = torch.zeros if len(live) < stride * stride else torch.empty
        dx = alloc(gy.shape[0], H, W, C, device=gy.device, dtype=gy.dtype)
    packed, offs = C_.conv_dgrad_wsub(w, [[r * S + s_ for _, r in tr for _, s_ in ts] for _, _, tr, ts in live])
    offs = offs.tolist()
    for i, (a, b, tr, ts) in enumerate(live):
        n = C * len(tr) * len(ts) * K
        wsub = packed[offs[i]:offs[i] + n].view(C, len(tr), len(ts), K)
        Hs, Ws = (H - a + stride - 1) // stride, (W - b + stride - 1) // stride
        C_.conv_fwd_subgrid(gy, wsub, -tr[0][0], Hs, Ws, dx, stride, a, b, *tail)
    if route == "parity_complete_sums":
        ln.complete(dx)
    elif route == "parity_relu_sums":
        ln.deposit(rsums, None, dx)
    return dx


def _plan_bwd(C_, gy, x, w, stride, padding, addend, xform, bn_link):
    K, R, S, C = w.shape
    if (xform is not None and addend is None and R == 1 and S == 1 and stride == 1 and padding == 0
            and os.environ.get("K8S_AMD_BWD1X1_FUSED", "1") != "0" and _link_kind(bn_link, x.shape) == "relu"
            and bn_link.x.data_ptr() == x.data_ptr() and gy.is_contiguous() and x.is_contiguous()
            and C_.bwd1x1_fused_ok(gy.numel() // K, C, K)):
        return "fused_1x1"
    if _hip(gy, x, w) and stride == 1 and K % 8 == 0 and C % 8 == 0:
        return "stride1"
    if _hip(gy, x, w) and strided_dgrad_ok(gy, w, stride, padding):
        return "strided"
    return "aten"


def _slot_written(p):
    p.store._notify(p) if p.written else p.store.mark_written(p)


def _finish_dw(p, gy, x, w, stride, padding):
    if p is not None:
        _vendor("wgrad", x, w, stride, padding)
        _, dw = _aten_bwd(gy, x, w, stride, padding, False, True)
        p.store.deposit(p, dw)


def conv_bwd(gy, x, w, stride, padding, need_dx, p=None, addend=None, xform=None, x_sub=None, bn_link=None):
    K, R, S, C = w.shape
    C_ = _load() if gy.is_cuda else None
    if x_sub is not None:
        _wgrad_hip(C_, gy, x_sub, p.grad.view(p.shape), 1, 0, p.written)
        STATS["hip_wgrad"] += 1
        _slot_written(p)
        p = None
    hip = _hip(gy, x, w)
    if xform is not None and not (hip and C % 64 == 0 and K % 8 == 0 and p is not None
                                  and p.grad.dtype == torch.float32):
        raise RuntimeError("normalize-on-load weight gradient outside the kernels' contract")
    if addend is not None and not torch.is_tensor(addend) and not (
            hip and stride == 1 and K % 8 == 0 and C % 8 == 0):
        addend = addend.materialize()
    family = _plan_bwd(C_, gy, x, w, stride, padding, addend, xform, bn_link) if need_dx else None
    if family == "fused_1x1":
        ROUTES[family] += 1
        STATS["hip_wgrad"] += 1
        STATS["hip_dgrad"] += 1
        sums = _bn_sums(C_, bn_link, C, gy.device)
        dz = C_.bwd1x1_fused(gy.view(-1, K), x.view(-1, C), w.view(K, C), xform, bn_link.gamma, bn_link.beta,
                             bn_link.mean, bn_link.invstd, p.grad.view(K, C), sums, p.written).view(x.shape)
        _slot_written(p)
        bn_link.deposit(sums, None, dz)
        return dz
    if hip and C % 8 == 0 and K % 8 == 0 and p is not None and p.grad.dtype == torch.float32:
        STATS["hip_wgrad"] += 1
        _wgrad_hip(C_, gy, x, p.grad.view(p.shape), stride, padding, p.written, xform)
        _slot_written(p)
        p = None
    dx = None
    if family in ("stride1", "strided"):
        STATS["hip_dgrad"] += 1
        if family == "stride1":
            dx = _dgrad_hip(C_, gy, w, padding, addend, bn_link)
        else:
            dx = _dgrad_strided_hip(C_, gy, w, stride, padding, x.shape[1], x.shape[2], addend, bn_link)
    elif family == "aten":
        ROUTES[family] += 1
        _vendor("dgrad", x, w, stride, padding)
        dx, _ = _aten_bwd(gy, x, w, stride, padding, True, False)
        if addend is not None:
            dx = dx + addend
    _finish_dw(p, gy, x, w, stride, padding)
    return dx


SUB1X1 = os.environ.get("K8S_AMD_SUB1X1", "1") != "0"


def subsample_ok(x, w, stride, padding) -> bool:
    K, R, S, C = w.shape
    return (SUB1X1 and stride > 1 and R == 1 and S == 1 and padding == 0 and _hip(x, w) and C % 64 == 0
            and K % 8 == 0 and x.is_contiguous())
```

k8s_amd/ops/nn.py:

```python
from __future__ import annotations

import os
from typing import Optional

import torch
import torch.nn.functional as F

from k8s_amd.ops import reference as ref
from k8s_amd.ops._ext import load as _load_ext


def _gpu(t: torch.Tensor) -> bool:
    return t.is_cuda


def _C():
    return _load_ext()


def _conv_impl():
    from k8s_amd.ops import conv as _conv

    return _conv


def _zero_scratch(store, device, n):
    from k8s_amd.parallel.flat import ZeroArena

    arena = store.__dict__.get("zero_arena")
    if arena is None or arena.device != torch.device(device):
        arena = store.zero_arena = ZeroArena(device)
    return arena.take(n)


class GradLink:
    __slots__ = ("grad", "shared")

    def __init__(self, shared: bool = False):
        self.grad = None
        self.shared = shared


class BiasLink:
    __slots__ = ("pb", "done")

    def __init__(self):
        self.pb, self.done = None, False


class ActLink:
    __slots__ = ("saved", "act", "pb", "done")

    def __init__(self):
        self.saved, self.act, self.pb, self.done = None, None, None, False


class SwiGLULink:
    __slots__ = ("saved", "dgu", "blk")

    def __init__(self, blk: int = 0):
        self.saved, self.dgu, self.blk = None, None, blk


class MaskedGrad:
    __slots__ = ("dy", "mask")

    def __init__(self, dy, mask):
        self.dy, self.mask = dy, mask

    def materialize(self):
        return _C().mask_apply(self.dy, self.mask)


class BnStatLink:
    __slots__ = ("kind", "x", "mask", "mean", "x2", "mean2", "invstd", "gamma", "beta", "sums", "sums2", "dy_key",
                 "store", "pending")

    def __init__(self):
        self.sums = self.sums2 = self.dy_key = None
        self.pending = False
        self._fill(None, None, None, None)

    def _fill(self, kind, store, x, mean, mask=None, x2=None, mean2=None, invstd=None, gamma=None, beta=None):
        self.kind, self.store = kind, store
        self.x, self.mean, self.mask, self.x2, self.mean2 = x, mean, mask, x2, mean2
        self.invstd, self.gamma, self.beta = invstd, gamma, beta

    def fill_relu(self, x, mean, invstd, gamma, beta, store=None):
        self._fill("relu", store, x, mean, invstd=invstd, gamma=gamma, beta=beta)

    def fill_mask(self, x, mask, mean, store=None):
        self._fill("mask", store, x, mean, mask)

    def fill_dual(self, x, mask, mean, x2, mean2, store=None):
        self._fill("dual", store, x, mean, mask, x2, mean2)

    def fill_pool(self, x, mask, mean, store=None):
        self._fill("pool", store, x, mean, mask)

    @staticmethod
    def _key(t):
        return t.data_ptr(), tuple(t.shape), t._version

    def deposit(self, sums, sums2, over):
        self.sums, self.sums2, self.dy_key = sums, sums2, self._key(over)
        _conv_impl().STATS["bn_bstats"] += 1

    def deposit_pending(self, sums):
        self.sums, self.sums2, self.dy_key, self.pending = sums, None, None, True
        _conv_impl().STATS["bn_bstats"] += 1

    def complete(self, over):
        self.dy_key, self.pending = self._key(over), False

    def drop_pending(self):
        self.sums, self.pending = None, False

    def covers(self, t) -> bool:
        return self.sums is not None and self.dy_key == self._key(t)

    def take(self, dy):
        pre = (self.sums, self.sums2) if self.covers(dy) else None
        self.sums = self.sums2 = self.dy_key = None
        self._fill(None, self.store, None, None)
        return pre


BN_BSTATS = os.environ.get("K8S_AMD_BN_BSTATS", "1") != "0"
BSTATS_POOL = os.environ.get("K8S_AMD_BN_BSTATS_POOL", "1") != "0"


class MaskLink:
    __slots__ = ("mask",)

    def __init__(self):
        self.mask = None


class _Conv2dNHWC(torch.autograd.Function):
    @staticmethod
    def forward(ctx, x, anchor, p, stride, padding, with_stats, link=None, bn_link=None):
        impl = _conv_impl()
        w = p.weight if x.dtype == p.weight.dtype else p.master.to(x.dtype)
        sums = None
        if with_stats and impl.fwd_uses_hip(x, w, stride, padding):
            sums = _zero_scratch(p.store, x.device, _C().conv_stat_replicas * 2 * w.shape[0]).view(
                _C().conv_stat_replicas, 2, w.shape[0])
        xs = None
        if impl.subsample_ok(x, w, stride, padding):
            xs = getattr(x, "_k8s_sub2", None) if stride == 2 else None
            if xs is None or xs.shape[:3] != ((x.shape[0], (x.shape[1] + 1) // 2, (x.shape[2] + 1) // 2)):
                xs = _C().subsample_nhwc(x, stride)
            y = impl.conv_fwd(xs, w, 1, 0, sums)
        else:
            y = impl.conv_fwd(x, w, stride, padding, sums)
        ctx.save_for_backward(x, xs)
        ctx.p, ctx.stride, ctx.padding, ctx.link, ctx.bn_link = p, stride, padding, link, bn_link
        ctx.x_requires_grad = x.requires_grad
        if sums is not None:
            ctx.mark_non_differentiable(sums)
        ctx.set_materialize_grads(False)
        return y, sums

    @staticmethod
    def backward(ctx, gy, _gsums=None):
        x, xs = ctx.saved_tensors
        p = ctx.p
        impl = _conv_impl()
        w = p.weight if x.dtype == p.weight.dtype else p.master.to(x.dtype)
        gy = gy.contiguous()
        addend = None
        if ctx.link is not None:
            addend, ctx.link.grad = ctx.link.grad, None
            if addend is None and ctx.link.shared and ctx.x_requires_grad:
                ctx.link.grad = impl.conv_bwd(gy, x, w, ctx.stride, ctx.padding, True, p, x_sub=xs,
                                              bn_link=ctx.bn_link)
                return None, None, None, None, None, None, None, None
        dx = impl.conv_bwd(gy, x, w, ctx.stride, ctx.padding, ctx.x_requires_grad, p, addend=addend, x_sub=xs,
                           bn_link=ctx.bn_link)
        return dx, None, None, None, None, None, None, None


def conv2d_nhwc(x: torch.Tensor, p, stride: int = 1, padding: int = 0, with_stats: bool = False,
                grad_link: "GradLink" = None):
    bn_link = getattr(x, "_k8s_bnstat", None)
    y, sums = _Conv2dNHWC.apply(x, p.store.anchor, p, stride, padding, with_stats, grad_link, bn_link)
    return (y, sums) if with_stats else y


def conv_bn_act_infer(x, pw, scale, shift, stride: int = 1, padding: int = 0, residual=None, relu: bool = True):
    assert not torch.is_grad_enabled(), "conv_bn_act_infer is an inference op: call it under torch.no_grad()"
    if torch.is_tensor(pw):
        w = pw
    else:
        w = pw.weight if x.dtype == pw.weight.dtype else pw.master.to(x.dtype)
    if _gpu(x):
        return _conv_impl().conv_infer(x, w, stride, padding, scale, shift, residual, relu)
    return ref.conv_bn_act_infer(x, w, scale, shift, stride, padding, residual, relu)


class _StemS2D(torch.autograd.Function):

    @staticmethod
    def forward(ctx, xs, anchor, p):
        C_ = _C()
        w7 = p.weight if p.weight.dtype == xs.dtype else p.master.to(xs.dtype)
        w4 = C_.stem_w_s2d(w7.contiguous())
        sums = _zero_scratch(p.store, xs.device, C_.conv_stat_replicas * 2 * w4.shape[0]).view(
            C_.conv_stat_replicas, 2, w4.shape[0])
        if tuple(w4.shape) == (64, 4, 4, 16) and (xs.shape[2] - 3) % 16 == 0 and xs.shape[2] - 3 <= 112:
            y = C_.stem_conv_fwd(xs.contiguous(), w4, sums)
        else:
            y = C_.conv_fwd(xs, w4, 1, 0, 1, False, None, 0, sums)
        _conv_impl().STATS["hip_fwd"] += 1
        ctx.save_for_backward(xs)
        ctx.p, ctx.kshape = p, tuple(w4.shape)
        ctx.mark_non_differentiable(sums)
        ctx.set_materialize_grads(False)
        return y, sums

    @staticmethod
    def backward(ctx, gy, _gsums=None):
        (xs,) = ctx.saved_tensors
        p, C_ = ctx.p, _C()
        dw4 = torch.empty(ctx.kshape, device=xs.device, dtype=torch.float32)
        if ctx.kshape == (64, 4, 4, 16) and (xs.shape[2] - 3) % 16 == 0 and xs.shape[2] - 3 <= 112:
            C_.stem_wgrad(xs.contiguous(), gy.contiguous(), dw4)
        else:
            _conv_impl()._wgrad_hip(C_, gy.contiguous(), xs, dw4, 1, 0, False)
        _conv_impl().STATS["hip_wgrad"] += 1
        dw7, finish = _param_grad(p, xs.device)
        C_.stem_dw_s2d(dw4, dw7)
        finish()
        return None, None, None


def stem_conv_s2d(xs, p):
    return _StemS2D.apply(xs, p.store.anchor, p)


def stem_s2d_input(images, pad: int = 3):
    return _C().stem_s2d_input(images.contiguous(), pad)


class _BnAct(torch.autograd.Function):
    @staticmethod
    def forward(ctx, x, res, anchor, pg, pb, run_mean, run_var, training, momentum, eps, relu, sums=None,
                res_link=None, dy_link=None, stat_link=None, sub2=None):
        x = x.contiguous()
        if res is not None:
            res = res.contiguous()
        want_mask = relu and res is not None and _gpu(x)
        mask = None
        want_sub = sub2 is not None and x.dim() == 4
        if _gpu(x) and sums is not None and training:
            out = _C().bn_fwd_from_sums(x, res, pg.master, pb.master, sums, run_mean, run_var, momentum, eps, relu,
                                        want_mask, want_sub)
            if want_sub:
                sub2.y = out[-1]
        elif _gpu(x):
            out = _C().bn_fwd(x, res, pg.master, pb.master, run_mean, run_var, training, momentum, eps, relu,
                              want_mask)
        else:
            out = ref.bn_fwd(x, res, pg.master, pb.master, run_mean, run_var, training, momentum, eps, relu)
        y, mean, invstd = out[0], out[1], out[2]
        if want_mask:
            mask = out[3]
        keep_y = relu and (res is not None or not _gpu(x)) and mask is None
        ctx.save_for_backward(x, y if keep_y else None, mean, invstd, mask)
        ctx.pg, ctx.pb, ctx.has_res, ctx.res_link = pg, pb, res is not None, res_link
        ctx.relu_x = relu and not keep_y and mask is None
        ctx.dy_link = dy_link if (dy_link is not None and not relu and res is None) else None
        ctx.stat_link = None
        if stat_link is not None and training and (mask is not None or ctx.relu_x):
            if mask is None:
                stat_link.fill_relu(x, mean, invstd, pg.master, pb.master, pg.store)
            else:
                stat_link.fill_mask(x, mask, mean, pg.store)
            ctx.stat_link = stat_link
        return y

    @staticmethod
    def backward(ctx, dy):
        x, y, mean, invstd, mask = ctx.saved_tensors
        pg, pb = ctx.pg, ctx.pb
        store = pg.store
        dy = dy.contiguous()
        if ctx.dy_link is not None and ctx.dy_link.mask is not None:
            mask, ctx.dy_link.mask = ctx.dy_link.mask, None
        mask_out = isinstance(ctx.res_link, MaskLink) and mask is not None and ctx.has_res
        if _gpu(x):
            dg, db, finish = _bn_param_grads(pg, pb, x.device)
            handoff = isinstance(ctx.res_link, GradLink) and ctx.has_res and mask is not None
            want_dres = ctx.has_res and not (handoff or mask_out)
            pre = ctx.stat_link.take(dy) if ctx.stat_link is not None else None
            if pre is not None and mask is None:
                dx, dres = _C().bn_bwd_relu_from_sums(dy, x, pre[0], mean, invstd, pg.master, pb.master, dg, db)[0], None
            elif pre is not None:
                dx, dres = _C().bn_bwd_from_sums(dy, x, mask, pre[0], mean, invstd, pg.master, pb.master, dg, db,
                                                 want_dres)
            else:
                dx, dres = _C().bn_bwd(dy, x, y, mean, invstd, pg.master, pb.master, ctx.relu_x, dg, db, want_dres,
                                       mask)
            if handoff:
                dres = MaskedGrad(dy, mask)
            elif mask_out:
                dres = dy
                ctx.res_link.mask = mask
            finish()
        else:
            dx, dres, dg, db = ref.bn_bwd(dy, x, y, mean, invstd, pg.master)
            store.deposit(pg, dg)
            store.deposit(pb, db)
        if ctx.has_res and isinstance(ctx.res_link, GradLink):
            ctx.res_link.grad, dres = dres, None
        return (dx, (dres if ctx.has_res else None), None, None, None, None, None, None, None, None, None, None, None,
                None, None, None)


BN_ONLOAD = os.environ.get("K8S_AMD_BN_ONLOAD", "1x1")
if BN_ONLOAD not in ("0", "1x1", "3x3"):
    raise ValueError("K8S_AMD_BN_ONLOAD must be 0 (BN applied by its own pass), 1x1 or 3x3, not %r" % BN_ONLOAD)


def _param_grad(p, device):
    slot = p.store.slot_for_write(p)
    g = slot.view(p.shape) if slot is not None else torch.empty(p.shape, device=device, dtype=torch.float32)
    return g, lambda: p.store.mark_written(p) if slot is not None else p.store.deposit(p, g)


def _bn_param_grads(pg, pb, device):
    (dg, finish_g), (db, finish_b) = _param_grad(pg, device), _param_grad(pb, device)
    return dg, db, lambda: (finish_g(), finish_b())


class _BnReluConv(torch.autograd.Function):

    @staticmethod
    def forward(ctx, x, sums, anchor, pg, pb, run_mean, run_var, momentum, eps, pw, stride, padding):
        C_ = _C()
        x = x.contiguous()
        M = x.numel() // x.shape[-1]
        mean, invstd, params = C_.bn_finalize(sums, pg.master, pb.master, run_mean, run_var, M, momentum, eps)
        w = pw.weight
        ysums = _zero_scratch(pw.store, x.device, C_.conv_stat_replicas * 2 * w.shape[0]).view(
            C_.conv_stat_replicas, 2, w.shape[0])
        y = C_.conv_fwd(x, w, stride, padding, 1, False, None, 0, ysums, xform=params)
        _conv_impl().STATS["hip_fwd"] += 1
        ctx.save_for_backward(x, mean, invstd, params)
        ctx.pg, ctx.pb, ctx.pw, ctx.stride, ctx.padding = pg, pb, pw, stride, padding
        ctx.x_requires_grad = x.requires_grad
        ctx.mark_non_differentiable(ysums)
        ctx.set_materialize_grads(False)
        return y, ysums

    @staticmethod
    def backward(ctx, gy, _gsums=None):
        x, mean, invstd, params = ctx.saved_tensors
        pg, pb, pw = ctx.pg, ctx.pb, ctx.pw
        impl = _conv_impl()
        gy = gy.contiguous()
        link = None
        if BN_BSTATS:
            link = BnStatLink()
            link.fill_relu(x, mean, invstd, pg.master, pb.master, pg.store)
        dz = impl.conv_bwd(gy, x, pw.weight, ctx.stride, ctx.padding, True, pw, xform=params, bn_link=link)
        dg, db, finish = _bn_param_grads(pg, pb, x.device)
        pre = link.take(dz) if link is not None else None
        if pre is not None:
            dx = _C().bn_bwd_relu_from_sums(dz, x, pre[0], mean, invstd, pg.master, pb.master, dg, db)[0]
        else:
            dx, _ = _C().bn_bwd(dz, x, None, mean, invstd, pg.master, pb.master, True, dg, db, False)
        finish()
        return (dx if ctx.x_requires_grad else None,) + (None,) * 11


ONLOAD_MAXC = int(os.environ.get("K8S_AMD_ONLOAD_MAXC", "128"))
ONLOAD3_MAXC = int(os.environ.get("K8S_AMD_ONLOAD3_MAXC", "0"))


def onload_ok(x, conv) -> bool:
    if BN_ONLOAD == "0" or x.shape[-1] > ONLOAD_MAXC:
        return False
    K_, R, S, C = conv.w.shape
    if R == 1 and S == 1:
        return conv.stride == 1 and conv.pad == 0
    return ((BN_ONLOAD == "3x3" or x.shape[-1] <= ONLOAD3_MAXC) and x.dim() == 4 and
            bool(_C().conv3x3_staged_ok(x.shape[1], x.shape[2], C, K_, R, S, conv.stride, conv.pad)))


def bn_relu_conv(t, bn, conv):
    x, sums = t if isinstance(t, tuple) else (t, None)
    w = conv.w
    if (sums is not None and bn.training and _gpu(x) and x.dtype == torch.bfloat16 and x.shape[-1] % 64 == 0
            and w.weight.dtype == torch.bfloat16 and w.shape[0] % 8 == 0 and w.grad.dtype == torch.float32
            and onload_ok(x, conv)):
        return _BnReluConv.apply(x, sums, w.store.anchor, bn.gamma, bn.beta, bn.running_mean, bn.running_var,
                                 bn.momentum, bn.eps, w, conv.stride, conv.pad)
    return conv(bn(t))


SUB2_FUSED = os.environ.get("K8S_AMD_SUB2_FUSED", "1") != "0"


class SubLink:
    __slots__ = ("y",)

    def __init__(self):
        self.y = None


def batch_norm_act(x, pg, pb, run_mean, run_var, residual=None, relu=True, training=True, momentum=0.1,
                   eps=1e-5, sums=None, res_link=None, dy_link=None, sub2=False):
    link = BnStatLink() if (BN_BSTATS and relu and training and _gpu(x)) else None
    sub = SubLink() if (sub2 and SUB2_FUSED and sums is not None and _gpu(x)) else None
    y = _BnAct.apply(x, residual, pg.store.anchor, pg, pb, run_mean, run_var, training, momentum, eps, relu,
                     sums, res_link, dy_link, link, sub)
    if link is not None and link.kind is not None:
        y._k8s_bnstat = link
    if sub is not None and sub.y is not None:
        y._k8s_sub2 = sub.y
    return y


class DropoutState:

    def __init__(self, seed: int = 0, device="cpu"):
        v = int(seed) & 0xFFFFFFFFFFFFFFFF
        self.tensor = torch.tensor([v - (1 << 64) if v >= (1 << 63) else v, 0], dtype=torch.int64, device=device)

    def to(self, device):
        self.tensor = self.tensor.to(device)
        return self

    def advance(self):
        self.tensor[1:2].add_(1)

    def set_step(self, n: int):
        self.tensor[1:2].fill_(int(n))

    @property
    def seed(self) -> int:
        return int(self.tensor[0]) & 0xFFFFFFFFFFFFFFFF

    @property
    def step(self) -> int:
        return int(self.tensor[1])


def _drop_spec(dropout, what):
    if dropout is None:
        return None
    p, state, site = dropout
    if not p:
        return None
    if not isinstance(state, DropoutState):
        raise TypeError("%s: dropout = (p, DropoutState, site)" % what)
    thr, scale = ref.drop_params(float(p))
    return float(p), thr, scale, state, int(site)


def _drop_fused(x) -> bool:
    return _gpu(x) and x.dtype == torch.bfloat16 and x.shape[-1] % 8 == 0


class _Dropout(torch.autograd.Function):
    @staticmethod
    def forward(ctx, x, spec):
        ctx.spec = spec
        return _Dropout._map(x.contiguous(), spec)

    @staticmethod
    def _map(x, spec):
        p, thr, scale, state, site = spec
        if _drop_fused(x):
            return _C().dropout(x, state.tensor, thr, scale, site)
        D = x.shape[-1]
        keep = ref.dropout_keep(state.tensor.to(x.device), site, x.numel() // D, D, p)
        return ref.dropout(x, keep, scale)

    @staticmethod
    def backward(ctx, dy):
        return _Dropout._map(dy.contiguous(), ctx.spec), None


def dropout(x, p: float, state: DropoutState, site: int):
    spec = _drop_spec((p, state, site), "dropout")
    return x if spec is None else _Dropout.apply(x, spec)


class _Norm(torch.autograd.Function):
    @staticmethod
    def forward(ctx, x, res, anchor, pg, pb, eps, rms, res_link=None, bias_link=None, drop=None):
        ctx.set_materialize_grads(False)
        x = x.contiguous()
        if res is not None:
            res = res.contiguous()
        beta = pb.master if pb is not None else None
        ctx.drop = drop
        if drop is not None:
            p, thr, scale, state, site = drop
            if _gpu(x):
                y, mean, rstd, xsum = _C().norm_fwd(x, res, pg.master, beta, eps, rms, state.tensor, thr, scale, site)
            else:
                D = x.shape[-1]
                keep = ref.dropout_keep(state.tensor, site, x.numel() // D, D, p)
                y, mean, rstd, xsum = ref.dropout_add_norm_fwd(x, res, pg.master, beta, eps, keep, scale)
        elif _gpu(x):
            y, mean, rstd, xsum = _C().norm_fwd(x, res, pg.master, beta, eps, rms)
        else:
            y, mean, rstd, xsum = ref.norm_fwd(x, res, pg.master, beta, eps, rms)
        xin = xsum if res is not None else x
        ctx.save_for_backward(xin, mean, rstd)
        ctx.pg, ctx.pb, ctx.rms, ctx.has_res = pg, pb, rms, res is not None
        ctx.res_link = res_link if res is not None else None
        ctx.bias_link = bias_link
        if res is not None:
            return y, xsum
        return y, None

    @staticmethod
    def backward(ctx, dy, dxsum):
        xin, mean, rstd = ctx.saved_tensors
        pg, pb = ctx.pg, ctx.pb
        store = pg.store
        if dy is None:
            dy = torch.zeros(xin.shape, device=xin.device, dtype=xin.dtype)
        dy = dy.contiguous()
        dres = dxsum.contiguous() if (dxsum is not None and ctx.has_res) else None
        drop, da = ctx.drop, None
        if _gpu(xin):
            sg = store.slot_for_write(pg)
            sb = store.slot_for_write(pb) if pb is not None else None
            dg = sg.view(pg.shape) if sg is not None else torch.empty(pg.shape, device=xin.device,
                                                                       dtype=torch.float32)
            db = None
            if pb is not None:
                db = sb.view(pb.shape) if sb is not None else torch.empty(pb.shape, device=xin.device,
                                                                           dtype=torch.float32)
            bl = ctx.bias_link
            lpb = bl.pb if (bl is not None and dres is None) else None
            dsum = None
            if lpb is not None:
                ss = store.slot_for_write(lpb) if lpb.store is store else None
                dsum = ss.view(lpb.shape) if ss is not None else torch.empty(lpb.shape, device=xin.device,
                                                                             dtype=torch.float32)
            if drop is not None:
                dx, da = _C().norm_bwd_dropout(dy, xin, pg.master, mean, rstd, dres, dg, db, dsum, drop[3].tensor,
                                               drop[1], drop[2], drop[4])
            else:
                dx = _C().norm_bwd(dy, xin, pg.master, mean, rstd, dres, dg, db, ctx.rms, dsum=dsum)
            store.mark_written(pg) if sg is not None else store.deposit(pg, dg)
            if pb is not None:
                store.mark_written(pb) if sb is not None else store.deposit(pb, db)
            if lpb is not None:
                lpb.store.mark_written(lpb) if ss is not None else lpb.store.deposit(lpb, dsum)
                bl.done = True
        else:
            if drop is not None:
                D = xin.shape[-1]
                keep = ref.dropout_keep(drop[3].tensor, drop[4], xin.numel() // D, D, drop[0])
                dx, da, dg, db, _ = ref.dropout_add_norm_bwd(dy, xin, pg.master, mean, rstd, dres, keep, drop[2])
            else:
                dx, dg, db = ref.norm_bwd(dy, xin, pg.master, mean, rstd, dres, ctx.rms)
            store.deposit(pg, dg)
            if pb is not None:
                store.deposit(pb, db)
        dres_out = None
        if ctx.has_res:
            dres_out = dx
            link = ctx.res_link
            if link is not None:
                if link.grad is None:
                    link.grad = dx
                    dres_out = None
                else:
                    dres_out = dx + link.grad
                    link.grad = None
        return (da if drop is not None else dx), dres_out, None, None, None, None, None, None, None, None


def layer_norm(x, pg, pb, eps=1e-12, residual=None, res_link=None, bias_link=None, dropout=None):
    drop = _drop_spec(dropout, "layer_norm")
    if drop is not None and residual is None:
        raise ValueError("layer_norm: dropout is applied to x on its way into the residual add; without a residual "
                         "use nn.dropout")
    y, xsum = _Norm.apply(x, residual, pg.store.anchor, pg, pb, eps, False, res_link, bias_link, drop)
    return (y, xsum) if residual is not None else y


def rms_norm(x, pg, eps=1e-5, residual=None, res_link=None):
    y, xsum = _Norm.apply(x, residual, pg.store.anchor, pg, None, eps, True, res_link)
    return (y, xsum) if residual is not None else y


def _gemm():
    from k8s_amd.ops import gemm as _g

    return _g


class _Linear(torch.autograd.Function):
    @staticmethod
    def forward(ctx, x, anchor, pw, pb, act, grad_link=None, bias_link=None, act_link=None, act_in=None,
                swiglu_in=None):
        g = _gemm()
        w = pw.weight if x.dtype == pw.weight.dtype else pw.master.to(x.dtype)
        x2 = x.reshape(-1, x.shape[-1])
        b = pb.master if pb is not None else None
        y, pre = g.linear_fwd(x2, w, b, act)
        ctx.save_for_backward(x2, pre)
        ctx.pw, ctx.pb, ctx.act, ctx.xshape, ctx.grad_link = pw, pb, act, x.shape, grad_link
        ctx.bias_link = bias_link
        if bias_link is not None and act is None:
            bias_link.pb = pb
        ctx.act_link = act_link if (act_link is not None and act is not None and pb is not None and
                                    pre is not None and pre.dtype == torch.bfloat16) else None
        if ctx.act_link is not None:
            act_link.saved, act_link.act, act_link.pb, act_link.done = pre, act, pb, False
        ctx.act_in = act_in
        ctx.swiglu_in = swiglu_in
        return y.reshape(*x.shape[:-1], w.shape[0])

    @staticmethod
    def backward(ctx, gy):
        x2, pre = ctx.saved_tensors
        pw, pb = ctx.pw, ctx.pb
        g = _gemm()
        w = pw.weight if x2.dtype == pw.weight.dtype else pw.master.to(x2.dtype)
        gy2 = gy.reshape(-1, gy.shape[-1]).contiguous()
        link = ctx.grad_link
        addend = None
        if link is not None and link.grad is not None:
            addend = link.grad.reshape(x2.shape)
            link.grad = None
        db_done = ctx.bias_link is not None and ctx.bias_link.done
        act = ctx.act
        if ctx.act_link is not None and ctx.act_link.done:
            ctx.act_link.done, ctx.act_link.saved = False, None
            act, db_done = None, True
        dx_act = None
        li = ctx.act_in
        if li is not None and li.saved is not None and g.dact_ok(x2, w, addend, gy):
            dx_act = (li.saved, li.act, li.pb, li.pb.store)
        sl, dx_swiglu = ctx.swiglu_in, None
        if dx_act is None and sl is not None and sl.saved is not None and g.swiglu_ok(x2, w, addend, gy):
            dx_swiglu = sl.saved
        dx, dw, db = g.linear_bwd(gy2, x2, w, pre, act, pw=pw, store=pw.store,
                                  need_db=pb is not None and not db_done, dx_addend=addend, pb=pb, dx_act=dx_act,
                                  dx_swiglu=dx_swiglu, swiglu_blk=sl.blk if dx_swiglu is not None else 0)
        if dx_act is not None:
            li.done, li.saved = True, None
        if dx_swiglu is not None:
            sl.dgu, sl.saved = dx, None
            dx = dx.new_zeros(()).expand(ctx.xshape)
        if dw is not None:
            pw.store.deposit(pw, dw)
        if pb is not None and db is not None:
            pb.store.deposit(pb, db)
        if link is not None and addend is None:
            link.grad = dx.reshape(ctx.xshape)
            return (None,) * 10
        return (dx.reshape(ctx.xshape),) + (None,) * 9


ACT_FUSE = True
SWIGLU_FUSE = os.environ.get("K8S_AMD_SWIGLU_FUSE", "1") != "0"


def linear(x, pw, pb=None, act: Optional[str] = None, grad_link=None, bias_link=None, act_link=None, act_in=None,
           swiglu_in=None):
    if not ACT_FUSE:
        act_link = act_in = None
    if not SWIGLU_FUSE:
        swiglu_in = None
    return _Linear.apply(x, pw.store.anchor, pw, pb, act, grad_link, bias_link, act_link, act_in, swiglu_in)


class _EmbeddingSum(torch.autograd.Function):

    @staticmethod
    def forward(ctx, anchor, S, dtype, *flat):
        ids = list(flat[0::2])
        pws = list(flat[1::2])
        T = next(i.numel() for i in ids if i is not None) if any(i is not None for i in ids) else None
        ws = [pw.weight if pw.weight.dtype == dtype else pw.master.to(dtype) for pw in pws]
        ids_c = [i.reshape(-1).contiguous() if i is not None else None for i in ids]
        out = _C().embed_fwd(ws, ids_c, T, S)
        ctx.save_for_backward(*[i if i is not None else torch.empty(0) for i in ids_c])
        ctx.has_ids = [i is not None for i in ids_c]
        ctx.pws, ctx.S = pws, S
        return out

    @staticmethod
    def backward(ctx, g):
        saved = ctx.saved_tensors
        ids = [t if h else None for t, h in zip(saved, ctx.has_ids)]
        g = g.contiguous()
        grads, finish = [], []
        for pw in ctx.pws:
            store = pw.store
            slot = store.slot_for_write(pw)
            if slot is not None:
                slot.zero_()
                grads.append(slot.view(pw.shape))
                finish.append(lambda pw=pw: pw.store.mark_written(pw))
            elif pw.grad.dtype == torch.float32:
                grads.append(pw.grad.view(pw.shape))
                finish.append(lambda pw=pw: pw.store._notify(pw))
            else:
                tmp = torch.zeros(pw.shape, device=g.device, dtype=torch.float32)
                grads.append(tmp)
                finish.append(lambda pw=pw, tmp=tmp: pw.store.deposit(pw, tmp))
        _C().embed_bwd(g, grads, ids, ctx.S)
        for f in finish:
            f()
        return (None, None, None) + (None,) * (2 * len(ctx.pws))


def embedding_sum(tables, S: int = 0, dtype=torch.bfloat16):
# ... 408 lines not shown
```

Before: 16320 images/s.

## Fuse bn3 BatchNorm backward apply into the bwd1x1 fused conv kernel load

Splits the masked BatchNorm backward into a params pass and an apply pass. The apply step (dx = sc*masked dy + B*x + D) for the bottleneck's third BN is folded into the tile loads of the following 1x1 fused backward kernel, so the dx tensor is never written and re-read. The kernel now stages gy, x3 and mask tiles in LDS and drops from three to two pipeline slots for the C=64 case. This adds LDS pressure and a barrier per stage, and the Python side needs link plumbing that falls back to a separate apply when the fused route is not taken.

```diff
diff --git a/k8s_amd/csrc/binding/batchnorm.cpp b/k8s_amd/csrc/binding/batchnorm.cpp
--- a/k8s_amd/csrc/binding/batchnorm.cpp
+++ b/k8s_amd/csrc/binding/batchnorm.cpp
@@ -211,6 +211,34 @@
   return bn_bwd_impl(dy, x, {}, mean, invstd, gamma, beta, false, dgamma, dbeta, want_dres, mask, &sums);
 }
 
+Tensor bn_bwd_params(Tensor dy, Tensor x, Tensor mask, OptTensor sums, Tensor mean, Tensor invstd, Tensor gamma,
+                     Tensor beta, Tensor dgamma, Tensor dbeta) {
+  const int C = bn_channels(x, "x", true);
+  const long M = x.numel() / C;
+  check_same_shape(dy, x, "dy");
+  check_bwd_vectors(mean, invstd, gamma, beta, dgamma, dbeta, C);
+  const uint8_t* mk = check_bit_mask(mask, x.numel(), "mask");
+  const bool pre = sums && sums->defined();
+  const int nrep = pre ? check_stat_sums(*sums, C, "sums", false) : 0;
+  auto params = torch::empty({4 * C}, gamma.options());
+  Tensor work;
+  if (!pre) work = torch::empty({k8s_amd::bn_workspace_floats(M, C)}, gamma.options());
+  launch_bn_bwd_params(cbf(dy), cbf(x), mk, pre ? f32(*sums) : nullptr, nrep, f32(mean), f32(invstd), f32(gamma),
+                       f32(beta), false, f32(dgamma), f32(dbeta), pre ? nullptr : f32(work), f32(params), M, C,
+                       cur_stream());
+  return params;
+}
+Tensor bn_bwd_apply(Tensor dy, Tensor x, Tensor mask, Tensor params) {
+  const int C = bn_channels(x, "x", true);
+  check_same_shape(dy, x, "dy");
+  const uint8_t* mk = check_bit_mask(mask, x.numel(), "mask");
+  check_channel_f32(params, 4L * C, "params");
+  TORCH_CHECK(params.device() == x.device(), "params: on x's device");
+  auto dx = torch::empty_like(x);
+  launch_bn_bwd_apply_pass(cbf(dy), cbf(x), mk, f32(params), false, bf(dx), nullptr, x.numel() / C, C, cur_stream());
+  return dx;
+}
+
 std::vector<Tensor> bn_bwd_dual_impl(const Tensor& dy, const Tensor& mask, const Tensor& x, const Tensor& mean,
                                      const Tensor& invstd, const Tensor& gamma, const Tensor& beta,
                                      const Tensor& dgamma, const Tensor& dbeta, const Tensor* sums, const Tensor& x2,
@@ -271,6 +299,10 @@
         "eps"_a);
   m.def("bn_bwd_relu_from_sums", &bn_bwd_relu_from_sums, "relu_x BatchNorm backward from a producer's sums");
   m.def("bn_bwd_from_sums", &bn_bwd_from_sums, "BatchNorm backward from a producer's reduction sums (final + apply)");
+  m.def("bn_bwd_params", &bn_bwd_params, "dy"_a, "x"_a, "mask"_a, "sums"_a, "mean"_a, "invstd"_a, "gamma"_a, "beta"_a,
+        "dgamma"_a, "dbeta"_a, "first half of a masked BatchNorm backward: dgamma, dbeta, params [sc | B | D | shift]");
+  m.def("bn_bwd_apply", &bn_bwd_apply, "dy"_a, "x"_a, "mask"_a, "params"_a,
+        "second half of a masked BatchNorm backward: dx from bn_bwd_params' table");
   m.def("bn_bwd_dual_from_sums", &bn_bwd_dual_from_sums, "bn_bwd_dual from a producer's reduction sums");
   m.def("bn_relu_maxpool", &bn_relu_maxpool, "x"_a, "sums"_a, "gamma"_a, "beta"_a, "run_mean"_a, "run_var"_a,
         "momentum"_a, "eps"_a, "want_link"_a = false);
diff --git a/k8s_amd/csrc/binding/conv.cpp b/k8s_amd/csrc/binding/conv.cpp
--- a/k8s_amd/csrc/binding/conv.cpp
+++ b/k8s_amd/csrc/binding/conv.cpp
@@ -95,7 +95,7 @@
 }
 
 Tensor bwd1x1_fused(Tensor gy, Tensor x, Tensor w, Tensor xform, Tensor gamma, Tensor beta, Tensor mean, Tensor invstd,
-                    Tensor dw, Tensor sums, bool accumulate) {
+                    Tensor dw, Tensor sums, bool accumulate, OptTensor x3, OptTensor mask, OptTensor params) {
   check_bf16_dense(gy, 2, "gy"); check_bf16_dense(x, 2, "x"); check_bf16_dense(w, 2, "w");
   const long M = gy.size(0), K = gy.size(1), C = x.size(1);
   TORCH_CHECK(x.size(0) == M && w.size(0) == K && w.size(1) == C, "shapes: gy [M, K], x [M, C], w [K, C]");
@@ -105,9 +105,24 @@
   TORCH_CHECK(dw.numel() == K * C, "dw must have K * C fp32 elements");
   check_channel_f32(xform, 2 * C, "xform (BatchNorm scale | shift)");
   const k8s_amd::BnBwdSums bb = bn_bwd_sums(x, mean, sums, {}, gamma, beta, invstd, {}, {}, {});
+  k8s_amd::Bwd1x1Bn3 bn3;
+  const bool onload = x3 || mask || params;
+  if (onload) {
+    TORCH_CHECK(x3 && mask && params, "bwd1x1_fused: x3, mask and params come together");
+    check_bf16_dense(*x3, 2, "x3");
+    TORCH_CHECK(x3->size(0) == M && x3->size(1) == K, "x3: the shape of gy, [M, K]");
+    bn3.mask = check_bit_mask(*mask, M * K, "mask");
+    check_aligned(*mask, "mask");
+    check_cuda(*params, "params"); check_dtype(*params, at::kFloat, "params"); check_aligned(*params, "params");
+    TORCH_CHECK(params->numel() >= 3 * K, "params: fp32 [sc | B | D], 3K elements or more");
+    TORCH_CHECK(x3->device() == gy.device() && mask->device() == gy.device() && params->device() == gy.device(),
+                "x3, mask and params: on gy's device");
+    bn3.x3 = cbf(*x3);
+    bn3.params = f32(*params);
+  }
   Tensor dz = torch::empty({M, C}, gy.options());
   launch_bwd1x1_fused(cbf(gy), cbf(x), cbf(w), f32(xform), bb.gamma, bb.beta, bb.mean, bb.invstd, bf(dz), f32(dw),
-                      bb.sums, M, (int)C, (int)K, accumulate, cur_stream());
+                      bb.sums, M, (int)C, (int)K, accumulate, cur_stream(), onload ? &bn3 : nullptr);
   return dz;
 }
 
@@ -192,7 +207,7 @@
   m.def("conv_wgrad", &conv_wgrad, "x"_a, "dy"_a, "dw"_a, "stride"_a, "pad"_a, "dil"_a, "splits"_a, "accumulate"_a,
         "xform"_a = py::none());
   m.def("bwd1x1_fused", &bwd1x1_fused, "gy"_a, "x"_a, "w"_a, "xform"_a, "gamma"_a, "beta"_a, "mean"_a, "invstd"_a,
-        "dw"_a, "sums"_a, "accumulate"_a,
+        "dw"_a, "sums"_a, "accumulate"_a, "x3"_a = py::none(), "mask"_a = py::none(), "params"_a = py::none(),
         "1x1 data gradient, normalize-on-load weight gradient and BatchNorm-backward sums in one pass (bwd1x1_fused.hip)");
   m.def("bwd1x1_fused_ok", [](int64_t M, int64_t C, int64_t K) {
     return C <= 1024 && K <= 4096 && k8s_amd::bwd1x1_fused_ok(M, (int)C, (int)K);
diff --git a/k8s_amd/csrc/kernels/batchnorm.hip b/k8s_amd/csrc/kernels/batchnorm.hip
--- a/k8s_amd/csrc/kernels/batchnorm.hip
+++ b/k8s_amd/csrc/kernels/batchnorm.hip
@@ -834,9 +834,14 @@
                      (int)relu_x, dx, dres, (int)nvec, C, make_fastdiv(C / 8), order);
 }
 
-void launch_bn_bwd(const uint16_t* dy, const uint16_t* x, const float* mean, const float* invstd, const float* gamma,
-                   const float* beta, bool relu_x, uint16_t* dx, uint16_t* dres, float* dgamma, float* dbeta,
-                   float* work, float* params, long M, int C, hipStream_t st, const uint8_t* mask) {
+void launch_bn_bwd_params(const uint16_t* dy, const uint16_t* x, const uint8_t* mask, const float* sums, int nrep,
+                          const float* mean, const float* invstd, const float* gamma, const float* beta, bool relu_x,
+                          float* dgamma, float* dbeta, float* work, float* params, long M, int C, hipStream_t st) {
+  if (sums) {
+    hipLaunchKernelGGL(bn_bwd_final_sums_kernel, dim3(cdiv(C, 256)), dim3(256), 0, st, sums, sums, nrep, C, dgamma,
+                       dbeta, 1.f / (float)M, mean, invstd, gamma, beta, params);
+    return;
+  }
   BnGeom g = bn_geom(C, M);
   const int nb = bn_reduce_blocks(M, g);
   const int rdir = stream_dir(1);
@@ -848,6 +853,18 @@
                        gamma, beta, (int)relu_x, M, C, g.tpr, g.rows_per_iter, work, mask, rdir);
   hipLaunchKernelGGL(bn_bwd_final_kernel, dim3(cdiv(C, FIN_CH)), dim3(256), 0, st, work, nb, C, dgamma, dbeta,
                      1.f / (float)M, mean, invstd, gamma, beta, params);
+}
+
+void launch_bn_bwd_apply_pass(const uint16_t* dy, const uint16_t* x, const uint8_t* mask, const float* params,
+                              bool relu_x, uint16_t* dx, uint16_t* dres, long M, int C, hipStream_t st) {
+  launch_bn_bwd_apply(dy, x, mask, params, relu_x, dx, dres, M, C, st);
+}
+
+void launch_bn_bwd(const uint16_t* dy, const uint16_t* x, const float* mean, const float* invstd, const float* gamma,
+                   const float* beta, bool relu_x, uint16_t* dx, uint16_t* dres, float* dgamma, float* dbeta,
+                   float* work, float* params, long M, int C, hipStream_t st, const uint8_t* mask) {
+  launch_bn_bwd_params(dy, x, mask, nullptr, 0, mean, invstd, gamma, beta, relu_x, dgamma, dbeta, work, params, M, C,
+                       st);
   launch_bn_bwd_apply(dy, x, mask, params, relu_x, dx, dres, M, C, st);
 }
 
@@ -855,8 +872,8 @@
                              const float* mean, const float* invstd, const float* gamma, const float* beta,
                              uint16_t* dx, uint16_t* dres, float* dgamma, float* dbeta, float* params, long M, int C,
                              hipStream_t st) {
-  hipLaunchKernelGGL(bn_bwd_final_sums_kernel, dim3(cdiv(C, 256)), dim3(256), 0, st, sums, sums, nrep, C, dgamma,
-                     dbeta, 1.f / (float)M, mean, invstd, gamma, beta, params);
+  launch_bn_bwd_params(dy, x, mask, sums, nrep, mean, invstd, gamma, beta, false, dgamma, dbeta, nullptr, params, M,
+                       C, st);
   launch_bn_bwd_apply(dy, x, mask, params, false, dx, dres, M, C, st);
 }
 
diff --git a/k8s_amd/csrc/kernels/bwd1x1_fused.hip b/k8s_amd/csrc/kernels/bwd1x1_fused.hip
--- a/k8s_amd/csrc/kernels/bwd1x1_fused.hip
+++ b/k8s_amd/csrc/kernels/bwd1x1_fused.hip
@@ -34,6 +34,9 @@
 
 struct Args {
   const uint16_t *gy, *x, *w;
+  const uint16_t* x3;
+  const uint8_t* mask;
+  const float* params;
   const float *xform, *gamma, *beta, *mean, *invstd;
   uint16_t* dz;
   float* dw;
@@ -47,19 +50,28 @@
   asm volatile("" ::: "memory");
 }
 
-template <int K, int RS, int NSLOT, int HALVES>
+template <int K, int RS, int NSLOT, int HALVES, bool ONLOAD>
 __global__ void __launch_bounds__(THREADS, 1) bwd1x1_fused_kernel(Args a) {
   constexpr int RB = K * 2, UG = K / 8;
-  constexpr int IMG_G = RS * RB, IMG_X = RS * 128, STAGE = IMG_G + IMG_X, RING = NSLOT * STAGE;
+  constexpr int IMG_G = RS * RB, IMG_X = RS * 128;
+  constexpr int IMG_M = ONLOAD ? RS * UG : 0;
+  constexpr int OFF_X = IMG_G + (ONLOAD ? IMG_G + IMG_M : 0);
+  constexpr int STAGE = OFF_X + IMG_X, RING = NSLOT * STAGE;
   constexpr int LG = RS * UG / THREADS;
+  constexpr int LPS = ONLOAD ? 2 * LG : LG;
+  constexpr bool TREG = ONLOAD && (THREADS / UG) % 16 == 0;
+  constexpr bool TLDS = ONLOAD && !TREG;
+  static_assert(!ONLOAD || (IMG_M % 1024 == 0 && IMG_M / 1024 <= THREADS / 64), "mask tile: whole 1-KB wave loads");
   constexpr int XT = RS * 8;
   constexpr int NKS = K / 32, KW = K / 8, KTW = KW / 16;
   static_assert(LG * THREADS == RS * UG && XT % 64 == 0 && XT <= THREADS && (RS == 32 || RS == 64), "tile");
   static_assert(XT * 64 <= RING, "sums partials reuse the ring");
   constexpr bool PLDS = K > 256;
-  __shared__ __attribute__((aligned(1024))) char smem[RING + IMG_X + (PLDS ? 5 * CT * 4 : 0)];
+  __shared__ __attribute__((aligned(1024))) char smem[RING + IMG_X + (PLDS ? 5 * CT * 4 : 0) + (TLDS ? 3 * K * 4 : 0)];
+  static_assert(sizeof(smem) <= 160 * 1024, "LDS");
   char* stg = smem + RING;
   float* ptab = reinterpret_cast<float*>(stg + IMG_X);
+  float* btab = ptab + (PLDS ? 5 * CT : 0);
 
   const int tid = threadIdx.x, lane = tid & 63;
   const int wid = __builtin_amdgcn_readfirstlane(tid >> 6);
@@ -112,6 +124,23 @@
       }
     }
   }
+  const int tup = tid % UG, trow = tid / UG;
+  float tsc[8], tB[8], tD[8];
+  if constexpr (TREG) {
+    const float* t = a.params + (tup ^ swz_g(trow)) * 8;
+#pragma unroll
+    for (int j = 0; j < 8; ++j) {
+      tsc[j] = t[j];
+      tB[j] = t[K + j];
+      tD[j] = t[2 * K + j];
+    }
+#pragma unroll
+    for (int j = 0; j < 8; ++j) asm volatile("" : "+v"(tsc[j]), "+v"(tB[j]), "+v"(tD[j]));
+  }
+  if constexpr (TLDS) {
+    static_assert(!TLDS || PLDS, "the table's stores are ordered by the PLDS barrier");
+    for (int i = tid; i < 3 * K; i += THREADS) btab[i] = a.params[i];
+  }
 #pragma unroll
   for (int ks = 0; ks < NKS; ++ks) asm volatile("" : "+v"(wf[ks]));
   if constexpr (!PLDS) {
@@ -124,6 +153,24 @@
   auto issue = [&](int slot, int i) {
     char* st = smem + slot * STAGE;
     const long m0 = (long)(pair + i * a.npairs) * RS;
+    if constexpr (ONLOAD) {
+      const unsigned last = (unsigned)min((long)RS - 1, M - 1 - m0);
+      const uint16_t* gb = a.gy + m0 * K;
+      const uint16_t* xb = a.x3 + m0 * K;
+#pragma unroll
+      for (int j = 0; j < LG; ++j) {
+        const unsigned row = j * (THREADS / UG) + trow;
+        const unsigned off = min(row, last) * K + (tup ^ swz_g(row)) * 8;
+        glds16(gb + off, st + j * (THREADS * 16) + wid * 1024);
+        glds16(xb + off, st + IMG_G + j * (THREADS * 16) + wid * 1024);
+      }
+      if (wid < IMG_M / 1024) {
+        const unsigned q = (wid * 64 + lane) * 16;
+        glds16(a.mask + m0 * UG + min(q / UG, last) * UG + q % UG, st + 2 * IMG_G + wid * 1024);
+      }
+      if (wid < XT / 64) glds16(a.x + m0 * C + min((unsigned)erow, last) * C + ecol, st + OFF_X + wid * 1024);
+      return;
+    }
 #pragma unroll
     for (int j = 0; j < LG; ++j) {
       const int sl = j * THREADS + tid, row = sl / UG, up = sl % UG;
@@ -135,7 +182,7 @@
     if (wid < XT / 64) {
       const long m = m0 + erow;
       const void* src = m < M ? (const void*)(a.x + m * C + ecol) : (const void*)g_zero16;
-      glds16(src, st + IMG_G + wid * 1024);
+      glds16(src, st + OFF_X + wid * 1024);
     }
   };
 
@@ -150,13 +197,48 @@
   int slot = 0;
   for (int s = 0; s < n; ++s) {
     const int younger = min(n - 1, s + NSLOT - 2) - s;
-    if (younger >= 2) asm volatile("s_waitcnt vmcnt(%0)" ::"n"(2 * LG) : "memory");
-    else if (younger == 1) asm volatile("s_waitcnt vmcnt(%0)" ::"n"(LG) : "memory");
+    if (younger >= 2) asm volatile("s_waitcnt vmcnt(%0)" ::"n"(2 * LPS) : "memory");
+    else if (younger == 1) asm volatile("s_waitcnt vmcnt(%0)" ::"n"(LPS) : "memory");
     else asm volatile("s_waitcnt vmcnt(0)" ::: "memory");
     lds_barrier();
     if (s + NSLOT - 1 < n) issue(slot == 0 ? NSLOT - 1 : slot - 1, s + NSLOT - 1);
     char* G = smem + slot * STAGE;
-    char* X = G + IMG_G;
+    char* X = G + OFF_X;
+
+    if constexpr (ONLOAD) {
+      const int last = (int)min((long)RS - 1, M - 1 - (long)(pair + s * a.npairs) * RS);
+#pragma unroll
+      for (int j = 0; j < LG; ++j) {
+        const int row = j * (THREADS / UG) + trow;
+        const int u = tup ^ swz_g(row);
+        char* gp = G + j * (THREADS * 16) + tid * 16;
+        const bf16x8_t gv = *reinterpret_cast<const bf16x8_t*>(gp);
+        const bf16x8_t xv = *reinterpret_cast<const bf16x8_t*>(gp + IMG_G);
+        const uint32_t bits = *reinterpret_cast<const uint8_t*>(G + 2 * IMG_G + row * UG + u);
+        float o[8];
+#pragma unroll
+        for (int h = 0; h < 8; h += 4) {
+          if constexpr (TLDS) {
+            const float* t = btab + u * 8 + h;
+#pragma unroll
+            for (int i = 0; i < 4; ++i) {
+              tsc[h + i] = t[i];
+              tB[h + i] = t[K + i];
+              tD[h + i] = t[2 * K + i];
+            }
+          }
+#pragma unroll
+          for (int i = h; i < h + 4; ++i) {
+            const float g = (bits >> i) & 1u ? bf2f((uint16_t)gv[i]) : 0.f;
+            o[i] = __builtin_fmaf(tsc[i], g, __builtin_fmaf(tB[i], bf2f((uint16_t)xv[i]), tD[i]));
+            o[i] = row <= last ? o[i] : 0.f;
+          }
+          if constexpr (TLDS) asm volatile("" ::: "memory");
+        }
+        *reinterpret_cast<bf16x8_t*>(gp) = pack_bf16x8(o);
+      }
+      lds_barrier();
+    }
 
     {
       f32x4_t d0 = {0.f, 0.f, 0.f, 0.f}, d1 = {0.f, 0.f, 0.f, 0.f};
@@ -288,22 +370,27 @@
 
 void launch_bwd1x1_fused(const uint16_t* gy, const uint16_t* x, const uint16_t* w, const float* xform,
                          const float* gamma, const float* beta, const float* mean, const float* invstd, uint16_t* dz,
-                         float* dw, float* sums, long M, int C, int K, bool accumulate, hipStream_t st) {
+                         float* dw, float* sums, long M, int C, int K, bool accumulate, hipStream_t st,
+                         const Bwd1x1Bn3* bn3) {
   using namespace b1f;
   if (!bwd1x1_fused_ok(M, C, K)) throw std::runtime_error("bwd1x1_fused: (C, K) = (64, 256) or (128, 512), M < 2^31");
+  if (bn3 && !(bn3->x3 && bn3->mask && bn3->params)) throw std::runtime_error("bwd1x1_fused: x3, mask and params");
   if (!accumulate) (void)hipMemsetAsync(dw, 0, (size_t)K * C * sizeof(float), st);
-  Args a{gy, x, w, xform, gamma, beta, mean, invstd, dz, dw, sums, (int)M, C, 0, 0};
+  Args a{gy, x, w, nullptr, nullptr, nullptr, xform, gamma, beta, mean, invstd, dz, dw, sums, (int)M, C, 0, 0};
+  if (bn3) a.x3 = bn3->x3, a.mask = bn3->mask, a.params = bn3->params;
   const int cus = std::max(1, planner_cus());
   if (C == 64) {
     a.ntiles = (int)((M + 63) / 64);
     a.npairs = cus;
-    hipLaunchKernelGGL((bwd1x1_fused_kernel<256, 64, 3, 1>), dim3(cus), dim3(THREADS), 0, st, a);
+    if (bn3) hipLaunchKernelGGL((bwd1x1_fused_kernel<256, 64, 2, 1, true>), dim3(cus), dim3(THREADS), 0, st, a);
+    else hipLaunchKernelGGL((bwd1x1_fused_kernel<256, 64, 3, 1, false>), dim3(cus), dim3(THREADS), 0, st, a);
   } else {
     const int grid = std::max(16, cus / 16 * 16);
     a.ntiles = (int)((M + 31) / 32);
     a.npairs = grid / 2;
-    hipLaunchKernelGGL((bwd1x1_fused_kernel<512, 32, 4, 2>), dim3(grid), dim3(THREADS), 0, st, a);
-  }
-}
-
-}
+    if (bn3) hipLaunchKernelGGL((bwd1x1_fused_kernel<512, 32, 2, 2, true>), dim3(grid), dim3(THREADS), 0, st, a);
+    else hipLaunchKernelGGL((bwd1x1_fused_kernel<512, 32, 4, 2, false>), dim3(grid), dim3(THREADS), 0, st, a);
+  }
+}
+
+}
diff --git a/k8s_amd/csrc/kernels/launchers.h b/k8s_amd/csrc/kernels/launchers.h
--- a/k8s_amd/csrc/kernels/launchers.h
+++ b/k8s_amd/csrc/kernels/launchers.h
@@ -79,6 +79,11 @@
 void launch_bn_bwd(const uint16_t* dy, const uint16_t* x, const float* mean, const float* invstd, const float* gamma,
                    const float* beta, bool relu_x, uint16_t* dx, uint16_t* dres, float* dgamma, float* dbeta,
                    float* work, float* params, long M, int C, hipStream_t st, const uint8_t* mask = nullptr);
+void launch_bn_bwd_params(const uint16_t* dy, const uint16_t* x, const uint8_t* mask, const float* sums, int nrep,
+                          const float* mean, const float* invstd, const float* gamma, const float* beta, bool relu_x,
+                          float* dgamma, float* dbeta, float* work, float* params, long M, int C, hipStream_t st);
+void launch_bn_bwd_apply_pass(const uint16_t* dy, const uint16_t* x, const uint8_t* mask, const float* params,
+                              bool relu_x, uint16_t* dx, uint16_t* dres, long M, int C, hipStream_t st);
 void launch_relu_mask(const uint16_t* y, uint8_t* mask, long nvec, hipStream_t st);
 
 void launch_norm_fwd(bool rms, const uint16_t* x, const uint16_t* res, uint16_t* xsum, const float* gamma,
@@ -196,10 +201,16 @@
 bool wgrad_stream_eligible(int N, int Ho, int Wo, int C, int K, int R, int S);
 void launch_wgrad_stream(const uint16_t* x, const uint16_t* dy, float* dw, int N, int H, int W, int C, int K, int R,
                          int S, int stride, int pad, int Ho, int Wo, bool accumulate, hipStream_t st);
+struct Bwd1x1Bn3 {
+  const uint16_t* x3 = nullptr;
+  const uint8_t* mask = nullptr;
+  const float* params = nullptr;
+};
 bool bwd1x1_fused_ok(long M, int C, int K);
 void launch_bwd1x1_fused(const uint16_t* gy, const uint16_t* x, const uint16_t* w, const float* xform,
                          const float* gamma, const float* beta, const float* mean, const float* invstd, uint16_t* dz,
-                         float* dw, float* sums, long M, int C, int K, bool accumulate, hipStream_t st);
+                         float* dw, float* sums, long M, int C, int K, bool accumulate, hipStream_t st,
+                         const Bwd1x1Bn3* bn3 = nullptr);
 void launch_conv_dgrad_wtrans(const uint16_t* w, uint16_t* w2, int K, int R, int S, int C, hipStream_t st);
 struct DgradTaps {
   int n[16];
diff --git a/k8s_amd/models/resnet.py b/k8s_amd/models/resnet.py
--- a/k8s_amd/models/resnet.py
+++ b/k8s_amd/models/resnet.py
@@ -19,13 +19,13 @@
         self.register_buffer("running_var", torch.ones(c))
         self.momentum, self.eps = 0.1, 1e-5
 
-    def forward(self, x, residual=None, relu=True, res_link=None, dy_link=None, sub2=False):
+    def forward(self, x, residual=None, relu=True, res_link=None, dy_link=None, sub2=False, bn3_link=None):
         sums = None
         if isinstance(x, tuple):
             x, sums = x
         return K.batch_norm_act(x, self.gamma, self.beta, self.running_mean, self.running_var, residual, relu,
                                 self.training, self.momentum, self.eps, sums=sums, res_link=res_link,
-                                dy_link=dy_link, sub2=sub2)
+                                dy_link=dy_link, sub2=sub2, bn3_link=bn3_link)
 
 
 class Conv(nn.Module):
@@ -69,13 +69,14 @@
                 idn = self.down_bn(dn, relu=False, dy_link=mlink)
         t = self.conv1(x, grad_link=link or dlink)
         t = K.bn_relu_conv(t, self.bn1, self.conv2)
-        t = K.bn_relu_conv(t, self.bn2, self.conv3)
+        b3 = K.Bn3Link() if (self.down is None and self.training) else None
+        t = K.bn_relu_conv(t, self.bn2, self.conv3, bn3_link=b3)
         if dn is not None and fuse:
             y = K.bn_act_dual(t, self.bn3, dn, self.down_bn)
             if y is not None:
                 return y
             idn = self.down_bn(dn, relu=False, dy_link=mlink)
-        return self.bn3(t, residual=idn, relu=True, res_link=link or mlink, sub2=sub2)
+        return self.bn3(t, residual=idn, relu=True, res_link=link or mlink, sub2=sub2, bn3_link=b3)
 
 
 class ResNet(nn.Module):
diff --git a/k8s_amd/ops/conv.py b/k8s_amd/ops/conv.py
--- a/k8s_amd/ops/conv.py
+++ b/k8s_amd/ops/conv.py
@@ -12,7 +12,8 @@
 
 
 STATS = {"hip_fwd": 0, "aten_fwd": 0, "hip_wgrad": 0, "aten_wgrad": 0, "hip_dgrad": 0, "aten_dgrad": 0,
-         "bn_bstats": 0, "hip_infer": 0, "aten_infer": 0}
+         "bn_bstats": 0, "hip_infer": 0, "aten_infer": 0,
+         "bn3_onload": 0, "bn3_apply": 0}
 ROUTES = collections.Counter()
 
 
@@ -297,9 +298,14 @@
         p.store.deposit(p, dw)
 
 
-def conv_bwd(gy, x, w, stride, padding, need_dx, p=None, addend=None, xform=None, x_sub=None, bn_link=None):
+def conv_bwd(gy, x, w, stride, padding, need_dx, p=None, addend=None, xform=None, x_sub=None, bn_link=None, bn3=None):
     K, R, S, C = w.shape
     C_ = _load() if gy.is_cuda else None
+    if bn3 is not None and not (need_dx and bn3.covers(gy)
+                                and _plan_bwd(C_, gy, x, w, stride, padding, addend, xform, bn_link) == "fused_1x1"):
+        STATS["bn3_apply"] += 1
+        gy = C_.bn_bwd_apply(gy.contiguous(), bn3.x3, bn3.mask, bn3.params)
+        bn3 = None
     if x_sub is not None:
         _wgrad_hip(C_, gy, x_sub, p.grad.view(p.shape), 1, 0, p.written)
         STATS["hip_wgrad"] += 1
@@ -315,11 +321,13 @@
     family = _plan_bwd(C_, gy, x, w, stride, padding, addend, xform, bn_link) if need_dx else None
     if family == "fused_1x1":
         ROUTES[family] += 1
+        STATS["bn3_onload"] += bn3 is not None
         STATS["hip_wgrad"] += 1
         STATS["hip_dgrad"] += 1
         sums = _bn_sums(C_, bn_link, C, gy.device)
+        onload = {} if bn3 is None else {"x3": bn3.x3.view(-1, K), "mask": bn3.mask, "params": bn3.params}
         dz = C_.bwd1x1_fused(gy.view(-1, K), x.view(-1, C), w.view(K, C), xform, bn_link.gamma, bn_link.beta,
-                             bn_link.mean, bn_link.invstd, p.grad.view(K, C), sums, p.written).view(x.shape)
+                             bn_link.mean, bn_link.invstd, p.grad.view(K, C), sums, p.written, **onload).view(x.shape)
         _slot_written(p)
         bn_link.deposit(sums, None, dz)
         return dz
diff --git a/k8s_amd/ops/nn.py b/k8s_amd/ops/nn.py
--- a/k8s_amd/ops/nn.py
+++ b/k8s_amd/ops/nn.py
@@ -135,6 +135,37 @@
 
     def __init__(self):
         self.mask = None
+
+
+def bn3_onload_on() -> bool:
+    return os.environ.get("K8S_AMD_BN3_ONLOAD", "1") != "0" and os.environ.get("K8S_AMD_BWD1X1_FUSED", "1") != "0"
+
+
+class Bn3Link:
+    __slots__ = ("y_key", "x3", "mask", "params", "dy_key")
+
+    def __init__(self):
+        self.y_key = self.x3 = self.mask = self.params = self.dy_key = None
+
+    def offer(self, y):
+        self.y_key = (y.data_ptr(), tuple(y.shape))
+
+    def offered(self, x) -> bool:
+        return self.y_key == (x.data_ptr(), tuple(x.shape))
+
+    def fill(self, dy, x3, mask, params):
+        self.x3, self.mask, self.params, self.dy_key = x3, mask, params, BnStatLink._key(dy)
+
+    def covers(self, t) -> bool:
+        return self.dy_key == BnStatLink._key(t)
+
+    def take(self):
+        if self.params is None:
+            return None
+        out = Bn3Link()
+        out.x3, out.mask, out.params, out.dy_key = self.x3, self.mask, self.params, self.dy_key
+        self.x3 = self.mask = self.params = self.dy_key = None
+        return out
 
 
 class _Conv2dNHWC(torch.autograd.Function):
@@ -246,7 +277,7 @@
 class _BnAct(torch.autograd.Function):
     @staticmethod
     def forward(ctx, x, res, anchor, pg, pb, run_mean, run_var, training, momentum, eps, relu, sums=None,
-                res_link=None, dy_link=None, stat_link=None, sub2=None):
+                res_link=None, dy_link=None, stat_link=None, sub2=None, bn3_link=None):
         x = x.contiguous()
         if res is not None:
             res = res.contiguous()
@@ -278,6 +309,8 @@
             else:
                 stat_link.fill_mask(x, mask, mean, pg.store)
             ctx.stat_link = stat_link
+        ctx.bn3_link = bn3_link if (bn3_link is not None and mask is not None and training
+                                    and bn3_link.offered(x)) else None
         return y
 
     @staticmethod
@@ -294,7 +327,12 @@
             handoff = isinstance(ctx.res_link, GradLink) and ctx.has_res and mask is not None
             want_dres = ctx.has_res and not (handoff or mask_out)
             pre = ctx.stat_link.take(dy) if ctx.stat_link is not None else None
-            if pre is not None and mask is None:
+            if ctx.bn3_link is not None and not want_dres and bn3_onload_on():
+                params = _C().bn_bwd_params(dy, x, mask, pre[0] if pre is not None else None, mean, invstd,
+                                            pg.master, pb.master, dg, db)
+                ctx.bn3_link.fill(dy, x, mask, params)
+                dx, dres = dy, None
+            elif pre is not None and mask is None:
                 dx, dres = _C().bn_bwd_relu_from_sums(dy, x, pre[0], mean, invstd, pg.master, pb.master, dg, db)[0], None
             elif pre is not None:
                 dx, dres = _C().bn_bwd_from_sums(dy, x, mask, pre[0], mean, invstd, pg.master, pb.master, dg, db,
@@ -302,6 +340,8 @@
             else:
                 dx, dres = _C().bn_bwd(dy, x, y, mean, invstd, pg.master, pb.master, ctx.relu_x, dg, db, want_dres,
                                        mask)
+            if ctx.bn3_link is not None and dx is not dy:
+                _conv_impl().STATS["bn3_apply"] += 1
             if handoff:
                 dres = MaskedGrad(dy, mask)
             elif mask_out:
@@ -315,7 +355,7 @@
         if ctx.has_res and isinstance(ctx.res_link, GradLink):
             ctx.res_link.grad, dres = dres, None
         return (dx, (dres if ctx.has_res else None), None, None, None, None, None, None, None, None, None, None, None,
-                None, None, None)
+                None, None, None, None)
 
 
 BN_ONLOAD = os.environ.get("K8S_AMD_BN_ONLOAD", "1x1")
@@ -337,7 +377,7 @@
 class _BnReluConv(torch.autograd.Function):
 
     @staticmethod
-    def forward(ctx, x, sums, anchor, pg, pb, run_mean, run_var, momentum, eps, pw, stride, padding):
+    def forward(ctx, x, sums, anchor, pg, pb, run_mean, run_var, momentum, eps, pw, stride, padding, bn3_link=None):
         C_ = _C()
         x = x.contiguous()
         M = x.numel() // x.shape[-1]
@@ -352,6 +392,12 @@
         ctx.x_requires_grad = x.requires_grad
         ctx.mark_non_differentiable(ysums)
         ctx.set_materialize_grads(False)
+        ctx.bn3_link = None
+        K_, R, S, C = w.shape
+        if (bn3_link is not None and BN_BSTATS and R == 1 and S == 1 and stride == 1 and padding == 0
+                and C_.bwd1x1_fused_ok(M, C, K_)):
+            bn3_link.offer(y)
+            ctx.bn3_link = bn3_link
         return y, ysums
 
     @staticmethod
@@ -364,7 +410,8 @@
         if BN_BSTATS:
             link = BnStatLink()
             link.fill_relu(x, mean, invstd, pg.master, pb.master, pg.store)
-        dz = impl.conv_bwd(gy, x, pw.weight, ctx.stride, ctx.padding, True, pw, xform=params, bn_link=link)
+        bn3 = ctx.bn3_link.take() if ctx.bn3_link is not None else None
+        dz = impl.conv_bwd(gy, x, pw.weight, ctx.stride, ctx.padding, True, pw, xform=params, bn_link=link, bn3=bn3)
         dg, db, finish = _bn_param_grads(pg, pb, x.device)
         pre = link.take(dz) if link is not None else None
         if pre is not None:
@@ -372,7 +419,7 @@
         else:
             dx, _ = _C().bn_bwd(dz, x, None, mean, invstd, pg.master, pb.master, True, dg, db, False)
         finish()
-        return (dx if ctx.x_requires_grad else None,) + (None,) * 11
+        return (dx if ctx.x_requires_grad else None,) + (None,) * 12
 
 
 ONLOAD_MAXC = int(os.environ.get("K8S_AMD_ONLOAD_MAXC", "128"))
@@ -389,14 +436,14 @@
             bool(_C().conv3x3_staged_ok(x.shape[1], x.shape[2], C, K_, R, S, conv.stride, conv.pad)))
 
 
-def bn_relu_conv(t, bn, conv):
+def bn_relu_conv(t, bn, conv, bn3_link=None):
     x, sums = t if isinstance(t, tuple) else (t, None)
     w = conv.w
     if (sums is not None and bn.training and _gpu(x) and x.dtype == torch.bfloat16 and x.shape[-1] % 64 == 0
             and w.weight.dtype == torch.bfloat16 and w.shape[0] % 8 == 0 and w.grad.dtype == torch.float32
             and onload_ok(x, conv)):
         return _BnReluConv.apply(x, sums, w.store.anchor, bn.gamma, bn.beta, bn.running_mean, bn.running_var,
-                                 bn.momentum, bn.eps, w, conv.stride, conv.pad)
+                                 bn.momentum, bn.eps, w, conv.stride, conv.pad, bn3_link)
     return conv(bn(t))
 
 
@@ -411,11 +458,11 @@
 
 
 def batch_norm_act(x, pg, pb, run_mean, run_var, residual=None, relu=True, training=True, momentum=0.1,
-                   eps=1e-5, sums=None, res_link=None, dy_link=None, sub2=False):
+                   eps=1e-5, sums=None, res_link=None, dy_link=None, sub2=False, bn3_link=None):
     link = BnStatLink() if (BN_BSTATS and relu and training and _gpu(x)) else None
     sub = SubLink() if (sub2 and SUB2_FUSED and sums is not None and _gpu(x)) else None
     y = _BnAct.apply(x, residual, pg.store.anchor, pg, pb, run_mean, run_var, training, momentum, eps, relu,
-                     sums, res_link, dy_link, link, sub)
+                     sums, res_link, dy_link, link, sub, bn3_link)
     if link is not None and link.kind is not None:
         y._k8s_bnstat = link
     if sub is not None and sub.y is not None:
```

Result: faster. 16710 images/s, median of 6 (+2.4%).
